# haosulab/ActiveZero

Measured on AMD Instinct MI355X. Metric: stereo pairs/sec (540x960, D=192) fwd+bwd, higher is better.
Workload: dtype f32; 1 GPU; configs[1]: PSMNet 540x960 (padded to 544 rows) D=192 fwd+bwd+Adam, supervised disparity loss, batch 4 per GPU; global_batch=4, height=540, width=960, maxdisp=192, parallelism=dp1

## Files before the change

activezero_amd/conv3d.py:

```python
import collections
import os

import torch

from . import _lib, overlap, packing, profiler
from .amax import AMAX_SLOTS, ZEROS, absmax, _get_amax, _set_amax, weight_amax
from .handover import slot_contribute, slot_leftover, slot_register, sum_parts
from .ops import _call, _chk, _p, _stream

CONV_S1, CONV_S2, DECONV_S2 = 0, 1, 2
FP32, BF16X6, F16X3 = 0, 1, 3
_PREC = {"fp32": FP32, "bf16x6": BF16X6, "f16x3": F16X3}
_BWD_F16 = os.environ.get("AZ_BWD_F16", "1") != "0"
PRESPLIT = os.environ.get("AZ_PRESPLIT", "1") != "0"
BF16X6_R16 = 2
_ROLL = os.environ.get("AZ_CONV_ROLL", "1") != "0"


_OFF32 = 0xffffff00


def _fits32(x, cin, cout):
    if isinstance(x, LazyCostVolume):
        return True
    _, d, h, w, _ = x.shape
    return d * h * w * max(cin, cout) * 4 < _OFF32


def _fits32_transposed(x, op_cin, op_cout):
    if not (op_cin == 64 and op_cout == 32):
        return True
    _, d, h, w, _ = x.shape
    return d * h * w * 64 * 4 < _OFF32 and 8 * d * h * w * 32 * 4 < _OFF32


def _layout(precision, mode, op_cout, fits32=True):
    if precision == BF16X6 and mode == CONV_S1 and op_cout == 32 and _ROLL and fits32:
        return BF16X6_R16
    return precision


def _fwd_launch(weight, mode):
    if mode == DECONV_S2:
        cin, cout = weight.shape[0], weight.shape[1]
        return cin, cout, 27, cout * 27
    cout, cin = weight.shape[0], weight.shape[1]
    return cin, cout, cin * 27, 27


def _dgrad_launch(mode, cin, cout):
    if mode == CONV_S1:
        return CONV_S1, cout, cin, 27, cin * 27, True
    if mode == CONV_S2:
        return DECONV_S2, cout, cin, 27, cin * 27, False
    return CONV_S2, cout, cin, cout * 27, 27, False


def _f16_fwd_ok(mode, cin, cout):
    return cin in (32, 64) and cout in (32, 64)


def _f16_dgrad_ok(mode, cin, cout):
    return _f16_fwd_ok(*_dgrad_launch(mode, cin, cout)[:3])


def _f16_wgrad_ok(mode, cin, cout):
    return cin in (32, 64) and cout in (32, 64)


def _f16_launch_ok(op_mode, ci, co, operand):
    if not _f16_fwd_ok(op_mode, ci, co):
        return False
    if op_mode == DECONV_S2:
        return _fits32_transposed(operand, ci, co)
    if _fits32(operand, ci, co):
        return True
    if op_mode == CONV_S1:
        return not (co == 32 or ci == co == 64)
    return not (ci == 32 and co == 64 and _lib.lib().az_option(b"AZ_CONV_S2ROLL") != 0)


class Arith(collections.namedtuple("Arith", "conv wgrad sink bwd16", defaults=(None, False))):
    __slots__ = ()

    @classmethod
    def of(cls, conv="bf16x6", wgrad=None, bwd16=None):
        w = wgrad if wgrad is not None else conv
        if bwd16 is None:
            bwd16 = _BWD_F16 or conv == "f16x3"
        return cls(_PREC[conv], BF16X6 if w == "f16x3" else _PREC[w], None, bool(bwd16) and conv != "fp32" and w != "fp32")

    @property
    def names(self):
        inv = {v: k for k, v in _PREC.items()}
        return inv[self.conv], ("f16x3" if self.bwd16 else inv[self.wgrad])


DEFAULT_ARITH = Arith.of(os.environ.get("AZ_CONV_PRECISION", "f16x3"), os.environ.get("AZ_WGRAD_PRECISION"))


def _arith(a):
    if a is None:
        return DEFAULT_ARITH
    if isinstance(a, str):
        return Arith.of(a)
    return a


def _dims(x):
    b, d, h, w, c = x.shape
    return b, d, h, w, c


def _out_dims(mode, d, h, w):
    if mode == CONV_S1:
        return d, h, w
    if mode == CONV_S2:
        return (d - 1) // 2 + 1, (h - 1) // 2 + 1, (w - 1) // 2 + 1
    return 2 * d, 2 * h, 2 * w


def _pack(weight, op_cin, op_cout, stride_out, stride_in, flip, precision, cache=False):
    w = _chk(weight.detach().contiguous(), "weight")

    def make():
        n = _lib.lib().az_conv3d_packed_floats(op_cin, op_cout, precision)
        packed = torch.empty(n, dtype=torch.float32, device=w.device)
        _call("az_conv3d_pack_weights", _p(packed), _p(w), op_cin, op_cout, stride_out, stride_in,
              int(flip), precision, _stream())
        packed.az_precision = precision
        return packed

    key = (packing.cache_key(weight), op_cin, op_cout, stride_out, stride_in, bool(flip), precision) if cache else None
    return packing.memo(packing.PACK_CACHE, key, make, (weight,), 256)


def eval_affine(bn, like, cache=False):
    c = bn.num_features
    src = (bn.weight, bn.bias, bn.running_mean, bn.running_var, bn.num_batches_tracked)

    def make():
        scale, shift = like.new_empty(c), like.new_empty(c)
        _call("az_bn3d_eval_affine", _p(scale), _p(shift), _p(bn.weight.detach()), _p(bn.bias.detach()),
              _p(bn.running_mean), _p(bn.running_var), float(bn.eps), c, _stream())
        return scale, shift

    return packing.memo(packing.AFFINE_CACHE, (packing.cache_key(*src), float(bn.eps)) if cache else None, make, src, 512)


def _pack_forward(weight, mode, precision, cache=False, lazy=False, fits32=True):
    cin, cout, s_out, s_in = _fwd_launch(weight, mode)
    if not lazy:
        precision = _layout(precision, mode, cout, fits32)
    return _pack(weight, cin, cout, s_out, s_in, False, precision, cache), cin, cout


def _peak(precision):
    if precision == F16X3:
        return _PEAK_F16
    return (157.3, "fp32 MFMA") if precision == FP32 else (2500.0 / 6.0, "bf16x6: bf16 MFMA peak / 6")


def _conv_flops(b, vox_out, cin, cout, mode):
    taps = 27.0 / 8.0 if mode == DECONV_S2 else 27.0
    return 2.0 * taps * cin * cout * b * vox_out


class LazyCostVolume:

    def __init__(self, feat_l_nhwc, feat_r_nhwc, ndisp):
        self.fl, self.fr, self.ndisp = _chk(feat_l_nhwc, "feat_l"), _chk(feat_r_nhwc, "feat_r"), int(ndisp)
        if self.fl.shape != self.fr.shape or self.fl.shape[-1] != 32:
            raise RuntimeError("fused cost volume expects two [B,h,w,32] feature maps")


def _run_gather(x, packed, mode, cin, cout, precision, scale=None, shift=None, residual=None, relu=False,
                stats=False, tag="conv3d"):
    if isinstance(x, LazyCostVolume):
        if stats or mode != CONV_S1 or cin != 64:
            raise RuntimeError("the fused cost-volume operand is only wired for the eval-mode dres0[0] conv")
        b, h, w, _ = x.fl.shape
        d = x.ndisp
        out = x.fl.new_empty(b, d, h, w, cout)
        with profiler.scope(f"{tag}_costvol_m0_{cin}_{cout}", flops=_conv_flops(b, d * h * w, cin, cout, mode),
                            peak=_peak(precision)):
            _call("az_conv3d_fwd", _p(out), _p(x.fl), _p(x.fr), _p(packed), _p(scale), _p(shift),
                  _p(residual), int(relu), mode, 1, getattr(packed, "az_precision", precision), b, cin, cout, d, h, w,
                  _stream())
        return out
    b, d, h, w, c = _dims(x)
    assert c == cin, (c, cin)
    precision = getattr(packed, "az_precision", precision)
    if mode == CONV_S2 and ((d % 2 and d != 1) or h % 2 or w % 2):
        raise RuntimeError("stride-2 layers need even D/H/W (as PSMNet's hourglass does; D = 1: a 2-D layer)")
    do, ho, wo = _out_dims(mode, d, h, w)
    out = x.new_empty(b, do, ho, wo, cout)
    flops = _conv_flops(b, do * ho * wo, cin, cout, mode)
    name = f"{tag}_m{mode}_{cin}_{cout}"
    if stats:
        ntiles = _lib.lib().az_conv3d_stats_tiles(mode, precision, b, cin, cout, d, h, w)
        if ntiles <= 0:
            raise RuntimeError(f"az_conv3d_stats_tiles: {ntiles}")
        part = x.new_empty(cout, ntiles, 2)
        cnt = x.new_empty(ntiles)
        with profiler.scope(name, flops=flops, peak=_peak(precision)):
            _call("az_conv3d_fwd_stats", _p(out), _p(part), _p(cnt), _p(x), None, _p(packed), mode, 0,
                  precision, b, cin, cout, d, h, w, _stream())
        return out, part, cnt, ntiles
    with profiler.scope(name, flops=flops, peak=_peak(precision)):
        _call("az_conv3d_fwd", _p(out), _p(x), None, _p(packed), _p(scale), _p(shift), _p(residual),
              int(relu), mode, 0, precision, b, cin, cout, d, h, w, _stream())
    return out


_PEAK_F16 = (2500.0 / 3.0, "f16x3: fp16 MFMA peak / 3")


def _pack_f16(weight, op_cin, op_cout, stride_out, stride_in, flip, mode, cache=False):
    w = _chk(weight.detach().contiguous(), "weight")

    def pack_now(packed, w_amax):
        _call("az_conv3d_pack_weights_f16", _p(packed), _p(w), _p(w_amax), op_cin, op_cout, stride_out, stride_in,
              int(flip), mode, _stream())

    def make():
        w_amax = weight_amax(weight, w)
        packed = torch.empty(_lib.lib().az_conv3d_packed_floats_f16(op_cin, op_cout), dtype=torch.float32, device=w.device)
        pack_now(packed, w_amax)
        return packed, w_amax

    if cache:
        key = (packing.cache_key(weight), op_cin, op_cout, stride_out, stride_in, bool(flip), F16X3, mode)
        return packing.memo(packing.PACK_CACHE, key, make, (weight,), 256)
    kind = _lib.lib().az_conv3d_f16_layout(mode, op_cin, op_cout)
    if kind < 0:
        raise RuntimeError(f"az_conv3d_f16_layout({mode}, {op_cin}, {op_cout}): {kind}")
    hit = packing.planned_pack(weight, w, kind, op_cin, op_cout, op_cin, op_cout, stride_out, stride_in, 27, flip, pack_now)
    return hit if hit is not None else make()


def _is_split(t):
    return getattr(t, "az_split", False)


def _run_f16(x, packed, w_amax, mode, cin, cout, scale=None, shift=None, residual=None, relu=False, stats=False,
             tag="conv3d"):
    b, d, h, w, c = _dims(x)
    assert c == cin, (c, cin)
    do, ho, wo = _out_dims(mode, d, h, w)
    out = x.new_empty(b, do, ho, wo, cout)
    name = f"{tag}_m{mode}_{cin}_{cout}"
    flops = _conv_flops(b, do * ho * wo, cin, cout, mode)
    split = _is_split(x)
    x_amax = _get_amax(x) if split else absmax(x)
    if split and (stats or x_amax is None):
        raise RuntimeError("a pre-split tensor reached a launch that cannot read it")
    if stats:
        ntiles = _lib.lib().az_conv3d_stats_tiles_f16(mode, b, cin, cout, d, h, w)
        if ntiles <= 0:
            raise RuntimeError(f"az_conv3d_stats_tiles_f16: {ntiles}")
        part, cnt = x.new_empty(cout, ntiles, 2), x.new_empty(ntiles)
        with profiler.scope(name, flops=flops, peak=_PEAK_F16):
            _call("az_conv3d_fwd_stats_f16", _p(out), _p(part), _p(cnt), _p(x), _p(packed), _p(x_amax), _p(w_amax),
                  mode, b, cin, cout, d, h, w, _stream())
        return out, part, cnt, ntiles
    with profiler.scope(name, flops=flops, peak=_PEAK_F16):
        _call("az_conv3d_fwd_f16", _p(out), _p(x), _p(packed), _p(x_amax), _p(w_amax), int(split), _p(scale), _p(shift),
              _p(residual), int(relu), mode, b, cin, cout, d, h, w, _stream())
    return out


def _conv(x, weight, mode, precision, scale=None, shift=None, residual=None, relu=False, stats=False, cache=False,
          tag="conv3d"):
    lazy = isinstance(x, LazyCostVolume)
    cin, cout, s_out, s_in = _fwd_launch(weight, mode)
    if precision == F16X3 and not lazy and _f16_launch_ok(mode, cin, cout, x):
        pk, w_amax = _pack_f16(weight, cin, cout, s_out, s_in, False, mode, cache)
        return _run_f16(x, pk, w_amax, mode, cin, cout, scale, shift, residual, relu, stats, tag)
    prec = BF16X6 if precision == F16X3 else precision
    packed, cin, cout = _pack_forward(weight, mode, prec, cache=cache, lazy=lazy, fits32=_fits32(x, cin, cout))
    return _run_gather(x, packed, mode, cin, cout, prec, scale, shift, residual, relu, stats, tag)


def _wgrad_f16(coarse, fine, stride, cm, cn, tag, sink=None, late_ok=True):
    b, dc, hc, wc, _ = _dims(coarse)
    _, df, hf, wf, _ = _dims(fine)
    gw = coarse.new_empty(cm, cn, 3, 3, 3)
    ws_bytes = _lib.lib().az_conv3d_wgrad_workspace(cm, cn)
    am_c, am_f = _get_amax(coarse), _get_amax(fine)
    mask = (1 if _is_split(coarse) else 0) | (2 if _is_split(fine) else 0)
    if (mask & 1 and am_c is None) or (mask & 2 and am_f is None):
        raise RuntimeError("a pre-split tensor without its producer's amax")
    with overlap.scope(sink, coarse, fine, gw, am_c, am_f):
        late = late_ok and sink is not None and sink.live and overlap.DEFER_UNPACK
        ws = sink.take_workspace(ws_bytes // 4) if late else coarse.new_empty(ws_bytes // 4)
        am_c = am_c if mask & 1 else absmax(coarse)
        am_f = am_f if mask & 2 else absmax(fine)
        with profiler.scope(f"{tag}_wgrad_s{stride}_{cm}_{cn}", flops=2.0 * 27 * cm * cn * b * dc * hc * wc,
                            peak=_PEAK_F16):
            _call("az_conv3d_wgrad_f16", None if late else _p(gw), _p(ws), ws_bytes, _p(coarse), _p(fine), _p(am_c), _p(am_f),
                  mask, stride, b, cm, cn, dc, hc, wc, df, hf, wf, _stream())
        if late:
            sink.defer_unpack(gw, ws, cm, cn, cm, cn, 27)
        if sink is not None and sink.live:
            sink.keep.extend((am_c, am_f))
    return gw


def _weight_grad_f16(x, dy, mode, cin, cout, sink=None, late_ok=True):
    if mode == DECONV_S2:
        return _wgrad_f16(x, dy, 2, cin, cout, "deconv", sink, late_ok)
    return _wgrad_f16(dy, x, 1 if mode == CONV_S1 else 2, cout, cin, "conv", sink, late_ok)


def _wgrad(coarse, fine, stride, cm, cn, tag, precision, sink=None):
    b, dc, hc, wc, _ = _dims(coarse)
    _, df, hf, wf, _ = _dims(fine)
    gw = coarse.new_empty(cm, cn, 3, 3, 3)
    ws_bytes = _lib.lib().az_conv3d_wgrad_workspace(cm, cn)
    with overlap.scope(sink, coarse, fine, gw):
        ws = coarse.new_empty(ws_bytes // 4)
        with profiler.scope(f"{tag}_wgrad_s{stride}_{cm}_{cn}", flops=2.0 * 27 * cm * cn * b * dc * hc * wc,
                            peak=_peak(precision)):
            _call("az_conv3d_wgrad", _p(gw), _p(ws), ws_bytes, _p(coarse), _p(fine), stride, precision,
                  b, cm, cn, dc, hc, wc, df, hf, wf, _stream())
    return gw


def _input_grad(dy, weight, mode, cin, cout, precision, residual=None):
    op, ci, co, s_out, s_in, flip = _dgrad_launch(mode, cin, cout)
    if precision == F16X3:
        if _f16_launch_ok(op, ci, co, dy):
            pk, w_amax = _pack_f16(weight, ci, co, s_out, s_in, flip, op)
            return _run_f16(dy, pk, w_amax, op, ci, co, residual=residual, tag="dgrad")
        precision = BF16X6
    pk = _pack(weight, ci, co, s_out, s_in, flip, _layout(precision, op, co, _fits32(dy, ci, co)))
    return _run_gather(dy, pk, op, ci, co, precision, residual=residual, tag="dgrad")


def _weight_grad(x, dy, mode, cin, cout, precision, sink=None, late_ok=True):
    if precision == F16X3:
        if _f16_wgrad_ok(mode, cin, cout):
            return _weight_grad_f16(x, dy, mode, cin, cout, sink, late_ok)
        precision = BF16X6
    if mode == DECONV_S2:
        return _wgrad(x, dy, 2, cin, cout, "deconv", precision, sink)
    return _wgrad(dy, x, 1 if mode == CONV_S1 else 2, cout, cin, "conv", precision, sink)


def _presplit_ok(x, raw, mode, cin, cout, need_gx, need_gw):
    lib = _lib.lib()
    b, d, h, w, _ = raw.shape
    if need_gx:
        op, ci, co = _dgrad_launch(mode, cin, cout)[:3]
        if not _f16_launch_ok(op, ci, co, raw) or lib.az_conv3d_fwd_f16_split_ok(op, b, ci, co, d, h, w) != 1:
            return False
    if need_gw:
        if not _f16_wgrad_ok(mode, cin, cout):
            return False
        _, dx_, hx, wx, _ = x.shape
        if mode == DECONV_S2:
            ok, bit = lib.az_conv3d_wgrad_f16_split_ok(2, b, cin, cout, dx_, hx, wx, d, h, w), 2
        else:
            ok, bit = lib.az_conv3d_wgrad_f16_split_ok(1 if mode == CONV_S1 else 2, b, cout, cin, d, h, w, dx_, hx, wx), 1
        if not ok & bit:
            return False
    return bool(need_gx or need_gw)


class _ConvBN(torch.autograd.Function):

    @staticmethod
    def forward(ctx, x, weight, gamma, beta, residual, bn, mode, relu, arith, defer=None, x_slot=None, res_slot=None):
        ctx.x_slot, ctx.res_slot = x_slot, res_slot
        x = _chk(x, "x")
        if residual is not None:
            residual = _chk(residual, "residual")
        training = bn.training or not bn.track_running_stats
        eps = float(bn.eps)
        cin, cout = _fwd_launch(weight, mode)[:2]
        with torch.cuda.device(x.device):
            if not training:
                scale, shift = eval_affine(bn, x)
                raw = _conv(x, weight, mode, arith.conv)
                y = torch.empty_like(raw)
                y_amax = ZEROS.take(raw)
                _call("az_bn3d_apply", _p(y), _p(raw), _p(scale), _p(shift), _p(residual), int(relu),
                      raw.numel() // cout, cout, _p(y_amax), _stream())
                _set_amax(y, y_amax)
                ctx.save_for_backward(x, weight, gamma, raw, y if relu else None, bn.running_mean.clone(),
                                      scale, None, None)
                ctx.cfg = (mode, relu, residual is not None, cin, cout, arith, False)
                return y
            raw, part, cnt, ntiles = _conv(x, weight, mode, arith.conv, stats=True)
            scale, shift = x.new_empty(cout), x.new_empty(cout)
            mean, invstd = x.new_empty(cout), x.new_empty(cout)
            track = bn.track_running_stats and bn.running_mean is not None
            momentum = 0.1 if bn.momentum is None else float(bn.momentum)
            nbt = bn.num_batches_tracked if (track and bn.num_batches_tracked is not None) else None
            scratch = x.new_empty(int(_lib.lib().az_bn3d_finalize_scratch(cout))) if ntiles >= 4096 else None
            _call("az_bn3d_finalize", _p(mean), _p(invstd), _p(scale), _p(shift),
                  _p(bn.running_mean) if track else None, _p(bn.running_var) if track else None,
                  _p(part), _p(cnt), _p(gamma.detach()), _p(beta.detach()), ntiles, cout, eps,
                  momentum, _p(nbt), _p(scratch), scratch.numel() if scratch is not None else 0, _stream())
            if nbt is not None:
                packing.touched(nbt, bn.running_mean, bn.running_var)
            nvox = raw.numel() // cout
            if defer is not None and relu and residual is None:
                defer.scale, defer.shift = scale, shift
                y = raw
            else:
                y = torch.empty_like(raw)
                y_amax = ZEROS.take(raw)
                with profiler.scope(f"bn3d_apply_{cout}", bytes=4.0 * raw.numel() * (3 if residual is not None else 2),
                                    bound="hbm"):
                    _call("az_bn3d_apply", _p(y), _p(raw), _p(scale), _p(shift), _p(residual), int(relu),
                          nvox, cout, _p(y_amax), _stream())
                _set_amax(y, y_amax)
        remask = relu and residual is None
        ctx.save_for_backward(x, weight, gamma, raw, y if (relu and not remask) else None, mean, invstd,
                              scale if remask else None, shift if remask else None)
        if arith.sink is not None and not arith.sink.owns(weight):
            arith = arith._replace(sink=None)
        ctx.cfg = (mode, relu, residual is not None, cin, cout, arith, True)
        ctx.x_amax = _get_amax(x)
        return y

    @staticmethod
    def backward(ctx, gy):
        x, weight, gamma, raw, y, mean, invstd, scale, shift = ctx.saved_tensors
        mode, relu, has_res, cin, cout, arith, training = ctx.cfg
        gy = _chk(gy.contiguous(), "grad_y")
        nvox = raw.numel() // cout
        with torch.cuda.device(gy.device):
            gy = slot_leftover(ctx, gy)
            if not training:
                s_, rm = invstd, mean
                dz = gy * (y > 0).to(gy.dtype) if relu else gy
                dbeta = dz.sum(dim=(0, 1, 2, 3))
                rinv = torch.where(gamma.detach() != 0, s_ / gamma.detach(), torch.zeros_like(s_))
                dgamma = (dz * (raw - rm)).sum(dim=(0, 1, 2, 3)) * rinv
                dx_raw = (dz * s_).contiguous()
                g_res = dz if has_res else None
            else:
                lib = _lib.lib()
                dx_raw = torch.empty_like(raw)
                dz = torch.empty_like(raw) if (has_res and relu) else None
                dgamma, dbeta = gy.new_empty(cout), gy.new_empty(cout)
                coef = gy.new_empty(cout, 3)
                ws_bytes = lib.az_bn3d_bwd_workspace(nvox, cout)
                ws = gy.new_empty(ws_bytes // 4)
                dx_amax = gy.new_empty(AMAX_SLOTS) if arith.bwd16 else None
                split = arith.bwd16 and PRESPLIT and _presplit_ok(x, raw, mode, cin, cout, ctx.needs_input_grad[0],
                                                                  ctx.needs_input_grad[1])
                with profiler.scope(f"bn3d_bwd_{cout}", bytes=4.0 * raw.numel() * (7 if (relu and y is not None) else 5), bound="hbm"):
                    _call("az_bn3d_bwd", _p(dx_raw), _p(dz), _p(dgamma), _p(dbeta), _p(coef), _p(ws), ws_bytes,
                          _p(gy), _p(y), _p(raw), _p(mean), _p(invstd), _p(gamma.detach()), _p(scale), _p(shift),
                          int(relu), nvox, cout, _p(dx_amax), int(split), _stream())
                if dx_amax is not None:
                    _set_amax(dx_raw, dx_amax)
                if split:
                    dx_raw.az_split = True
                g_res = (dz if relu else gy) if has_res else None
            gx = gw = None
            if has_res:
                g_res = slot_contribute(ctx.res_slot, plain=g_res)
            if ctx.needs_input_grad[0]:
                gx = slot_contribute(ctx.x_slot, make=lambda r: _input_grad(dx_raw, weight, mode, cin, cout,
                                                                             F16X3 if arith.bwd16 else arith.conv, r))
            if ctx.needs_input_grad[1]:
                if getattr(ctx, "x_amax", None) is not None and _get_amax(x) is None:
                    _set_amax(x, ctx.x_amax)
                gw = _weight_grad(x, dx_raw, mode, cin, cout, F16X3 if arith.bwd16 else arith.wgrad, arith.sink)
        return gx, gw, dgamma, dbeta, g_res, None, None, None, None, None, None, None


class DeferredAffine:

    def __init__(self):
        self.scale = self.shift = None

    @property
    def pending(self):
        return self.scale is not None


def conv_bn(x, conv, bn, mode, relu=False, residual=None, arith=None, defer=None):
    arith = _arith(arith)
    if isinstance(x, LazyCostVolume):
        if torch.is_grad_enabled() or bn.training:
            raise RuntimeError("LazyCostVolume is an inference-only operand")
        with torch.cuda.device(x.fl.device):
            scale, shift = eval_affine(bn, x.fl, cache=True)
            return _conv(x, conv.weight, mode, arith.conv, scale, shift, residual, relu, cache=True)
    training = bn.training or not bn.track_running_stats
    if not training and not torch.is_grad_enabled():
        x = _chk(x, "x")
        with torch.cuda.device(x.device):
            scale, shift = eval_affine(bn, x, cache=True)
            return _conv(x, conv.weight, mode, arith.conv, scale, shift,
                         _chk(residual, "residual") if residual is not None else None, relu, cache=True)
    w = arith.sink.weight(conv.weight) if arith.sink is not None else conv.weight
    x_slot = slot_register(x)
    res_slot = slot_register(residual) if residual is not None else None
    return _ConvBN.apply(x, w, bn.weight, bn.bias, residual, bn, mode, relu, arith, defer, x_slot, res_slot)


class _ConvLogits(torch.autograd.Function):

    @staticmethod
    def forward(ctx, x, weight, addend, sink, scale=None, shift=None):
        ctx.sink = sink if (sink is not None and sink.owns(weight)) else None
        x = _chk(x, "x")
        w = _chk(weight.detach().contiguous(), "weight")
        b, d, h, wd, c = _dims(x)
        if c != 32 or tuple(w.shape) != (1, 32, 3, 3, 3):
            raise RuntimeError("classifier conv expects 32 -> 1 channels, 3x3x3")
        if addend is not None:
            addend = _chk(addend.contiguous(), "addend")
        out = x.new_empty(b, d, h, wd)
        with torch.cuda.device(x.device):
            with profiler.scope("conv3d_c1_fwd", bytes=4.0 * (x.numel() + out.numel()), bound="hbm"):
                _call("az_conv3d_c1_fwd", _p(out), _p(x), _p(w), _p(addend), _p(scale), _p(shift), b, d, h, wd, _stream())
        ctx.save_for_backward(x, w, scale, shift)
        ctx.has_add = addend is not None
        return out

    @staticmethod
    def backward(ctx, g):
        x, w, scale, shift = ctx.saved_tensors
        g = _chk(g.contiguous(), "grad_logits")
        b, d, h, wd, _ = _dims(x)
        gx = gw = None
        with torch.cuda.device(g.device):
            if ctx.needs_input_grad[0]:
                gx = torch.empty_like(x)
                with profiler.scope("conv3d_c1_dgrad", bytes=4.0 * (x.numel() + g.numel()), bound="hbm"):
                    _call("az_conv3d_c1_dgrad", _p(gx), _p(g), _p(w), b, d, h, wd, _stream())
            if ctx.needs_input_grad[1]:
                gw = torch.empty_like(w)
                with overlap.scope(ctx.sink, x, g, gw, scale, shift), \
                        profiler.scope("conv3d_c1_wgrad", bytes=4.0 * (x.numel() + g.numel()), bound="hbm"):
                    _call("az_conv3d_c1_wgrad", _p(gw), _p(x), _p(g), _p(scale), _p(shift), b, d, h, wd, _stream())
        return gx, gw, (g if ctx.has_add else None), None, None, None


def conv_logits(x, conv, addend=None, sink=None, affine=None):
    sc, sh = (affine.scale, affine.shift) if (affine is not None and affine.pending) else (None, None)
    return _ConvLogits.apply(x, sink.weight(conv.weight) if sink is not None else conv.weight, addend, sink, sc, sh)


class _AddRelu(torch.autograd.Function):
    @staticmethod
    def forward(ctx, a, b):
        a, b = _chk(a, "a"), _chk(b, "b")
        y = torch.empty_like(a)
        y_amax = ZEROS.take(a)
        with torch.cuda.device(a.device):
            _call("az_add_relu", _p(y), _p(a), _p(b), 0, a.numel(), _p(y_amax), _stream())
        _set_amax(y, y_amax)
        return y

    @staticmethod
    def backward(ctx, g):
        return g, g


def add(a, b):
    return _AddRelu.apply(a, b)


class _FanOut(torch.autograd.Function):

    @staticmethod
    def forward(ctx, x, n):
        views = tuple(x.view_as(x) for _ in range(n))
        am = _get_amax(x)
        if am is not None:
            for v in views:
                _set_amax(v, am)
        return views

    @staticmethod
    def backward(ctx, *grads):
        gs = [_chk(g.contiguous(), "grad") for g in grads if g is not None]
        if not gs:
            return None, None
        with torch.cuda.device(gs[0].device):
            return sum_parts(gs), None


def fanout(x, n):
    if not (torch.is_grad_enabled() and x.requires_grad) or x.numel() % 4:
        return (x,) * n
    return _FanOut.apply(x, n)


def conv_plain(x, weight, mode, arith=None):
    arith = _arith(arith)
    return _conv(_chk(x, "x"), weight, mode, arith.conv)
```

activezero_amd/csrc/az_bn3d.hip:

```cpp
#include <stdlib.h>

#include "az_roll_common.h"

__device__ __forceinline__ double bn_wave_sum(double v) {
#pragma unroll
    for (int o = 32; o > 0; o >>= 1) v += __shfl_xor(v, o);
    return v;
}
template <int NT>
__device__ __forceinline__ double bn_block_sum(double v, double *slots ) {
    v = bn_wave_sum(v);
    __syncthreads();
    if ((threadIdx.x & 63) == 0) slots[threadIdx.x >> 6] = v;
    __syncthreads();
    double t = 0.0;
#pragma unroll
    for (int w = 0; w < NT / 64; ++w) t += slots[w];
    return t;
}

#define BN_PRE_SLICES 32
__global__ void __launch_bounds__(256)
bn_premerge_kernel(float *__restrict__ part_out, float *__restrict__ cnt_out, const float *__restrict__ part,
                   const float *__restrict__ cnt, long long ntiles) {
    const int c = blockIdx.x, sl = blockIdx.y;
    const long long per = (ntiles + BN_PRE_SLICES - 1) / BN_PRE_SLICES;
    const long long t0 = sl * per, t1 = t0 + per < ntiles ? t0 + per : ntiles;
    __shared__ double slots[256 / 64];
    const float2 *pc = reinterpret_cast<const float2 *>(part) + (long long)c * ntiles;
    double n = 0.0, sum = 0.0;
    for (long long t = t0 + threadIdx.x; t < t1; t += 256) {
        n += (double)cnt[t];
        sum += (double)pc[t].x;
    }
    const double N = bn_block_sum<256>(n, slots);
    const double S = bn_block_sum<256>(sum, slots);
    const double mean = N > 0.0 ? S / N : 0.0;
    double m2 = 0.0;
    for (long long t = t0 + threadIdx.x; t < t1; t += 256) {
        const float nt = cnt[t];
        if (nt <= 0.f) continue;
        const float2 pr = pc[t];
        const double dlt = (double)pr.x / (double)nt - mean;
        m2 += (double)pr.y + (double)nt * dlt * dlt;
    }
    const double M2 = bn_block_sum<256>(m2, slots);
    if (threadIdx.x == 0) {
        reinterpret_cast<float2 *>(part_out)[c * BN_PRE_SLICES + sl] = make_float2((float)S, (float)M2);
        if (c == 0) cnt_out[sl] = (float)N;
    }
}

#define BN_FIN_THREADS 1024
__global__ void __launch_bounds__(BN_FIN_THREADS)
bn_finalize_kernel(float *__restrict__ mean_out, float *__restrict__ invstd_out,
                   float *__restrict__ scale, float *__restrict__ shift,
                   float *__restrict__ running_mean, float *__restrict__ running_var,
                   const float *__restrict__ part, const float *__restrict__ cnt,
                   const float *__restrict__ gamma, const float *__restrict__ beta,
                   long long ntiles, int C, float eps, float momentum, int groups,
                   long long *__restrict__ num_batches_tracked) {
    const int c = blockIdx.x;
    if (num_batches_tracked != nullptr && c == 0 && threadIdx.x == 0) *num_batches_tracked += groups;
    for (int grp = 0; grp < groups; ++grp, part += (long long)C * ntiles * 2, cnt += ntiles,
             mean_out += C, invstd_out += C, scale += C, shift += C) {
    __shared__ double slots[BN_FIN_THREADS / 64];
    const float2 *pc = reinterpret_cast<const float2 *>(part) + (long long)c * ntiles;
    double n = 0.0, sum = 0.0;
    for (long long t = threadIdx.x; t < ntiles; t += BN_FIN_THREADS) {
        n += (double)cnt[t];
        sum += (double)pc[t].x;
    }
    const double Ntot = bn_block_sum<BN_FIN_THREADS>(n, slots);
    const double mean_all = bn_block_sum<BN_FIN_THREADS>(sum, slots) / Ntot;
    double m2 = 0.0;
    for (long long t = threadIdx.x; t < ntiles; t += BN_FIN_THREADS) {
        const float nt = cnt[t];
        if (nt <= 0.f) continue;
        const float2 pr = pc[t];
        const double dlt = (double)pr.x / (double)nt - mean_all;
        m2 += (double)pr.y + (double)nt * dlt * dlt;
    }
    const double M2 = bn_block_sum<BN_FIN_THREADS>(m2, slots);
    if (threadIdx.x == 0) {
        const double N = Ntot, mu = mean_all, var = M2 / N;
        const double istd = 1.0 / sqrt(var + (double)eps);
        mean_out[c] = (float)mu;
        invstd_out[c] = (float)istd;
        const float sc = gamma[c] * (float)istd;
        scale[c] = sc;
        shift[c] = beta[c] - (float)mu * sc;
        if (running_mean) {
            const double unbiased = N > 1.0 ? M2 / (N - 1.0) : var;
            running_mean[c] = (1.f - momentum) * running_mean[c] + momentum * (float)mu;
            running_var[c] = (1.f - momentum) * running_var[c] + momentum * (float)unbiased;
        }
    }
    }
}

__global__ void bn_eval_affine_kernel(float *scale, float *shift, const float *gamma,
                                      const float *beta, const float *rm, const float *rv,
                                      float eps, int C) {
    const int c = blockIdx.x * blockDim.x + threadIdx.x;
    if (c >= C) return;
    const float sc = gamma[c] / sqrtf(rv[c] + eps);
    scale[c] = sc;
    shift[c] = beta[c] - rm[c] * sc;
}

typedef float az_v4f __attribute__((ext_vector_type(4)));
template <bool NT>
__device__ __forceinline__ float4 bn_ld4(const float4 *p) {
    if (NT) {
        const az_v4f v = __builtin_nontemporal_load(reinterpret_cast<const az_v4f *>(p));
        return make_float4(v[0], v[1], v[2], v[3]);
    }
    return *p;
}
template <bool NT>
__device__ __forceinline__ void bn_st4(float4 *p, const float4 &o) {
    if (NT) {
        const az_v4f v = {o.x, o.y, o.z, o.w};
        __builtin_nontemporal_store(v, reinterpret_cast<az_v4f *>(p));
    } else {
        *p = o;
    }
}
#define BN_NT_BYTES (256LL << 20)

template <int C, bool NT>
__global__ void __launch_bounds__(256)
bn_apply_kernel(float4 *__restrict__ y, const float4 *__restrict__ x,
                const float *__restrict__ scale, const float *__restrict__ shift,
                const float4 *__restrict__ res, int relu, long long total4, unsigned *__restrict__ amax = nullptr) {
    constexpr int C4 = C / 4;
    unsigned am = 0;
    __shared__ float4 ssc[C4], ssh[C4];
    {
        const long long go = (long long)blockIdx.y * total4;
        y += go; x += go; if (res) res += go;
        scale += blockIdx.y * C; shift += blockIdx.y * C;
    }
    if (threadIdx.x < C4) {
        ssc[threadIdx.x] = reinterpret_cast<const float4 *>(scale)[threadIdx.x];
        ssh[threadIdx.x] = reinterpret_cast<const float4 *>(shift)[threadIdx.x];
    }
    __syncthreads();
    for (long long i = blockIdx.x * 256LL + threadIdx.x; i < total4; i += gridDim.x * 256LL) {
        const int c4 = (int)(i % C4);
        const float4 v = bn_ld4<NT>(&x[i]), sc = ssc[c4], sh = ssh[c4];
        float4 o = make_float4(fmaf(v.x, sc.x, sh.x), fmaf(v.y, sc.y, sh.y), fmaf(v.z, sc.z, sh.z),
                               fmaf(v.w, sc.w, sh.w));
        if (res) {
            const float4 r = bn_ld4<NT>(&res[i]);
            o.x += r.x; o.y += r.y; o.z += r.z; o.w += r.w;
        }
        if (relu) {
            o.x = fmaxf(o.x, 0.f); o.y = fmaxf(o.y, 0.f); o.z = fmaxf(o.z, 0.f); o.w = fmaxf(o.w, 0.f);
        }
        bn_st4<NT>(&y[i], o);
        az_amax_acc(am, o);
    }
    if (amax) az_amax_flush(amax, am);
}

__device__ __forceinline__ int c4_of(int tid, int C4) { return tid % C4; }

template <int C, bool NT>
__global__ void __launch_bounds__(256)
bn_bwd_reduce_kernel(float *__restrict__ partial, const float *__restrict__ dy,
                     const float *__restrict__ y, const float *__restrict__ x,
                     const float *__restrict__ mean, const float *__restrict__ invstd,
                     const float *__restrict__ scale, const float *__restrict__ shift, int relu,
                     long long nvox, unsigned *__restrict__ amax_zero = nullptr, unsigned *__restrict__ pmax = nullptr) {
    if (amax_zero && blockIdx.x == 0 && blockIdx.y == 0 && threadIdx.x < AZ_AMAX_SLOTS) amax_zero[threadIdx.x * AZ_AMAX_STRIDE] = 0u;
    constexpr int C4 = C / 4, VPB = 256 / C4;
    const bool remask = relu && scale != nullptr;
    {
        const long long go = (long long)blockIdx.y * nvox * C;
        dy += go; x += go; if (relu && !remask) y += go;
        mean += blockIdx.y * C; invstd += blockIdx.y * C;
        if (remask) { scale += blockIdx.y * C; shift += blockIdx.y * C; }
        partial += (size_t)blockIdx.y * gridDim.x * C * 2;
    }
    float4 sc = make_float4(0, 0, 0, 0), sh = sc;
    if (remask) { sc = reinterpret_cast<const float4 *>(scale)[c4_of(threadIdx.x, C4)]; sh = reinterpret_cast<const float4 *>(shift)[c4_of(threadIdx.x, C4)]; }
    const int c4 = threadIdx.x % C4, vl = threadIdx.x / C4;
    const float4 mu = reinterpret_cast<const float4 *>(mean)[c4];
    const float4 is = reinterpret_cast<const float4 *>(invstd)[c4];
    float4 s1 = make_float4(0, 0, 0, 0), s2 = make_float4(0, 0, 0, 0);
    uint4 mg = make_uint4(0, 0, 0, 0), mx = make_uint4(0, 0, 0, 0);
    auto body = [&](const float4 gin, const float4 xx, const float4 yin, float4 &t1, float4 &t2) {
        float4 g = gin;
        if (relu) {
            float4 yy = yin;
            if (remask) yy = make_float4(fmaf(xx.x, sc.x, sh.x), fmaf(xx.y, sc.y, sh.y), fmaf(xx.z, sc.z, sh.z), fmaf(xx.w, sc.w, sh.w));
            g.x = yy.x > 0.f ? g.x : 0.f; g.y = yy.y > 0.f ? g.y : 0.f;
            g.z = yy.z > 0.f ? g.z : 0.f; g.w = yy.w > 0.f ? g.w : 0.f;
        }
        const float4 xh = make_float4((xx.x - mu.x) * is.x, (xx.y - mu.y) * is.y, (xx.z - mu.z) * is.z, (xx.w - mu.w) * is.w);
        t1.x += g.x; t1.y += g.y; t1.z += g.z; t1.w += g.w;
        t2.x += g.x * xh.x; t2.y += g.y * xh.y; t2.z += g.z * xh.z; t2.w += g.w * xh.w;
        if (pmax) {
            mg.x = max(mg.x, az_finite_abs_bits(g.x)); mg.y = max(mg.y, az_finite_abs_bits(g.y));
            mg.z = max(mg.z, az_finite_abs_bits(g.z)); mg.w = max(mg.w, az_finite_abs_bits(g.w));
            mx.x = max(mx.x, az_finite_abs_bits(xh.x)); mx.y = max(mx.y, az_finite_abs_bits(xh.y));
            mx.z = max(mx.z, az_finite_abs_bits(xh.z)); mx.w = max(mx.w, az_finite_abs_bits(xh.w));
        }
    };
    const long long stride = (long long)gridDim.x * VPB;
    float4 u1 = make_float4(0, 0, 0, 0), u2 = make_float4(0, 0, 0, 0);
    const float4 zero4 = make_float4(0, 0, 0, 0);
    long long v = (long long)blockIdx.x * VPB + vl;
    for (; v + stride < nvox; v += 2 * stride) {
        const size_t i = (size_t)v * C4 + c4, i2 = (size_t)(v + stride) * C4 + c4;
        const float4 ga = bn_ld4<NT>(reinterpret_cast<const float4 *>(dy) + i), gb = bn_ld4<NT>(reinterpret_cast<const float4 *>(dy) + i2);
        const float4 xa = bn_ld4<NT>(reinterpret_cast<const float4 *>(x) + i), xb = bn_ld4<NT>(reinterpret_cast<const float4 *>(x) + i2);
        float4 ya = zero4, yb = zero4;
        if (relu && !remask) { ya = bn_ld4<NT>(reinterpret_cast<const float4 *>(y) + i); yb = bn_ld4<NT>(reinterpret_cast<const float4 *>(y) + i2); }
        body(ga, xa, ya, s1, s2);
        body(gb, xb, yb, u1, u2);
    }
    if (v < nvox) {
        const size_t i = (size_t)v * C4 + c4;
        const float4 ga = bn_ld4<NT>(reinterpret_cast<const float4 *>(dy) + i), xa = bn_ld4<NT>(reinterpret_cast<const float4 *>(x) + i);
        float4 ya = zero4;
        if (relu && !remask) ya = bn_ld4<NT>(reinterpret_cast<const float4 *>(y) + i);
        body(ga, xa, ya, s1, s2);
    }
    s1.x += u1.x; s1.y += u1.y; s1.z += u1.z; s1.w += u1.w;
    s2.x += u2.x; s2.y += u2.y; s2.z += u2.z; s2.w += u2.w;
    static_assert(C4 <= 64 && 64 % C4 == 0, "channel quads must tile a wave");
#pragma unroll
    for (int off = C4; off < 64; off <<= 1) {
        s1.x += __shfl_xor(s1.x, off); s1.y += __shfl_xor(s1.y, off); s1.z += __shfl_xor(s1.z, off); s1.w += __shfl_xor(s1.w, off);
        s2.x += __shfl_xor(s2.x, off); s2.y += __shfl_xor(s2.y, off); s2.z += __shfl_xor(s2.z, off); s2.w += __shfl_xor(s2.w, off);
    }
    __shared__ float4 r1[4][C4], r2[4][C4];
    const int wave = threadIdx.x >> 6, lane = threadIdx.x & 63;
    if (lane < C4) { r1[wave][lane] = s1; r2[wave][lane] = s2; }
    __syncthreads();
    if (threadIdx.x < C4) {
#pragma unroll
        for (int k = 1; k < 4; ++k) {
            const float4 a = r1[k][c4], b = r2[k][c4];
            s1.x += a.x; s1.y += a.y; s1.z += a.z; s1.w += a.w;
            s2.x += b.x; s2.y += b.y; s2.z += b.z; s2.w += b.w;
        }
        float *p = partial + ((size_t)blockIdx.x * C + c4 * 4) * 2;
        p[0] = s1.x; p[1] = s2.x; p[2] = s1.y; p[3] = s2.y;
        p[4] = s1.z; p[5] = s2.z; p[6] = s1.w; p[7] = s2.w;
    }
    if (pmax) {
#pragma unroll
        for (int off = C4; off < 64; off <<= 1) {
            mg.x = max(mg.x, (unsigned)__shfl_xor((int)mg.x, off)); mg.y = max(mg.y, (unsigned)__shfl_xor((int)mg.y, off));
            mg.z = max(mg.z, (unsigned)__shfl_xor((int)mg.z, off)); mg.w = max(mg.w, (unsigned)__shfl_xor((int)mg.w, off));
            mx.x = max(mx.x, (unsigned)__shfl_xor((int)mx.x, off)); mx.y = max(mx.y, (unsigned)__shfl_xor((int)mx.y, off));
            mx.z = max(mx.z, (unsigned)__shfl_xor((int)mx.z, off)); mx.w = max(mx.w, (unsigned)__shfl_xor((int)mx.w, off));
        }
        __shared__ uint4 q1[4][C4], q2[4][C4];
        if (lane < C4) { q1[wave][lane] = mg; q2[wave][lane] = mx; }
        __syncthreads();
        if (threadIdx.x < C4) {
#pragma unroll
            for (int k = 1; k < 4; ++k) {
                const uint4 a = q1[k][c4], b = q2[k][c4];
                mg.x = max(mg.x, a.x); mg.y = max(mg.y, a.y); mg.z = max(mg.z, a.z); mg.w = max(mg.w, a.w);
                mx.x = max(mx.x, b.x); mx.y = max(mx.y, b.y); mx.z = max(mx.z, b.z); mx.w = max(mx.w, b.w);
            }
            unsigned *p = pmax + ((size_t)blockIdx.y * gridDim.x * C + (size_t)blockIdx.x * C + c4 * 4) * 2;
            p[0] = mg.x; p[1] = mx.x; p[2] = mg.y; p[3] = mx.y;
            p[4] = mg.z; p[5] = mx.z; p[6] = mg.w; p[7] = mx.w;
        }
    }
}

#define BN_BWD_PARTIAL_FLOATS 32768
template <int C, bool NT>
__global__ void __launch_bounds__(256)
bn_bwd_apply_kernel(float4 *__restrict__ dx, float4 *__restrict__ dz_out,
                    const float4 *__restrict__ dy, const float4 *__restrict__ y,
                    const float4 *__restrict__ x, const float *__restrict__ mean,
                    const float *__restrict__ invstd, float *__restrict__ coef,
                    const float *__restrict__ scale, const float *__restrict__ shift, int relu,
                    long long total4, const float *__restrict__ partial, int nblocks, const float *__restrict__ gamma,
                    float *__restrict__ dgamma, float *__restrict__ dbeta, double nvox,
                    unsigned *__restrict__ amax = nullptr, const unsigned *__restrict__ pmax = nullptr) {
    constexpr int C4 = C / 4;
    unsigned am = 0;
    float split_scale = 1.f;
    __shared__ float smu[C], sis[C], k0[C], k1[C], k2[C], ssc[C], ssh[C];
    const bool remask = relu && scale != nullptr;
    const int grp = blockIdx.y;
    {
        const long long go = (long long)grp * total4;
        dx += go; dy += go; x += go; if (relu && !remask) y += go; if (dz_out) dz_out += go;
        mean += grp * C; invstd += grp * C; coef += grp * C * 3;
        if (remask) { scale += grp * C; shift += grp * C; }
    }
    if (remask && threadIdx.x < C) { ssc[threadIdx.x] = scale[threadIdx.x]; ssh[threadIdx.x] = shift[threadIdx.x]; }
    if (threadIdx.x < C) {
        smu[threadIdx.x] = mean[threadIdx.x];
        sis[threadIdx.x] = invstd[threadIdx.x];
    }
    constexpr int COLS = C / 2, ROWS = 256 / COLS;
    static_assert(COLS <= 64 && 64 % COLS == 0, "a partial row must tile a wave");
    __shared__ float wsum[4][2 * C];
    const int j = threadIdx.x % COLS, r = threadIdx.x / COLS, wave = threadIdx.x >> 6;
    const bool writer = blockIdx.x == 0;
    const int g_lo = (writer && grp == 0) ? 0 : grp, g_hi = (writer && grp == 0) ? (int)gridDim.y : grp + 1;
    double dg_tot = 0.0, db_tot = 0.0;
    for (int g = g_lo; g < g_hi; ++g) {
        const float4 *p4 = reinterpret_cast<const float4 *>(partial) + (size_t)g * nblocks * COLS;
        double a0 = 0.0, a1 = 0.0, a2 = 0.0, a3 = 0.0;
        for (int blk = r; blk < nblocks; blk += ROWS) {
            const float4 v = p4[(size_t)blk * COLS + j];
            a0 += v.x; a1 += v.y; a2 += v.z; a3 += v.w;
        }
#pragma unroll
        for (int off = COLS; off < 64; off <<= 1) {
            a0 += __shfl_xor(a0, off); a1 += __shfl_xor(a1, off); a2 += __shfl_xor(a2, off); a3 += __shfl_xor(a3, off);
        }
        __syncthreads();
        if ((threadIdx.x & 63) < COLS) {
            wsum[wave][4 * j + 0] = (float)a0; wsum[wave][4 * j + 1] = (float)a1;
            wsum[wave][4 * j + 2] = (float)a2; wsum[wave][4 * j + 3] = (float)a3;
        }
        __syncthreads();
        if (threadIdx.x < C) {
            const int c = threadIdx.x;
            const double sa = ((double)wsum[0][2 * c] + (double)wsum[1][2 * c]) + ((double)wsum[2][2 * c] + (double)wsum[3][2 * c]);
            const double sb = ((double)wsum[0][2 * c + 1] + (double)wsum[1][2 * c + 1]) + ((double)wsum[2][2 * c + 1] + (double)wsum[3][2 * c + 1]);
            db_tot += sa; dg_tot += sb;
            if (g == grp) {
                k0[c] = gamma[c] * sis[c];
                k1[c] = (float)(sa / nvox);
                k2[c] = (float)(sb / nvox);
                if (writer) { coef[c * 3 + 0] = k0[c]; coef[c * 3 + 1] = k1[c]; coef[c * 3 + 2] = k2[c]; }
            }
        }
    }
    if (writer && grp == 0 && threadIdx.x < C) { dbeta[threadIdx.x] = (float)db_tot; dgamma[threadIdx.x] = (float)dg_tot; }
    if (pmax) {
        const uint4 *m4 = reinterpret_cast<const uint4 *>(pmax);
        uint4 m = make_uint4(0, 0, 0, 0);
        for (int blk = r; blk < nblocks; blk += ROWS) {
            const uint4 v = m4[(size_t)blk * COLS + j];
            m.x = max(m.x, v.x); m.y = max(m.y, v.y); m.z = max(m.z, v.z); m.w = max(m.w, v.w);
        }
#pragma unroll
        for (int off = COLS; off < 64; off <<= 1) {
            m.x = max(m.x, (unsigned)__shfl_xor((int)m.x, off)); m.y = max(m.y, (unsigned)__shfl_xor((int)m.y, off));
            m.z = max(m.z, (unsigned)__shfl_xor((int)m.z, off)); m.w = max(m.w, (unsigned)__shfl_xor((int)m.w, off));
        }
        __syncthreads();
        if ((threadIdx.x & 63) < COLS) {
            wsum[wave][4 * j + 0] = __uint_as_float(m.x); wsum[wave][4 * j + 1] = __uint_as_float(m.y);
            wsum[wave][4 * j + 2] = __uint_as_float(m.z); wsum[wave][4 * j + 3] = __uint_as_float(m.w);
        }
        __syncthreads();
        float bnd = 0.f;
        if (threadIdx.x < C) {
            const int c = threadIdx.x;
            const float gm = fmaxf(fmaxf(wsum[0][2 * c], wsum[1][2 * c]), fmaxf(wsum[2][2 * c], wsum[3][2 * c]));
            const float xm = fmaxf(fmaxf(wsum[0][2 * c + 1], wsum[1][2 * c + 1]), fmaxf(wsum[2][2 * c + 1], wsum[3][2 * c + 1]));
            bnd = fabsf(k0[c]) * (gm + fabsf(k1[c]) + xm * fabsf(k2[c])) * 1.000001f;
            bnd = bnd < __builtin_inff() ? bnd : 0.f;
        }
#pragma unroll
        for (int off = 32; off > 0; off >>= 1) bnd = fmaxf(bnd, __shfl_xor(bnd, off));
        __shared__ float bwave[4];
        if ((threadIdx.x & 63) == 0) bwave[wave] = bnd;
        __syncthreads();
        bnd = fmaxf(fmaxf(bwave[0], bwave[1]), fmaxf(bwave[2], bwave[3]));
        split_scale = az_pow2(az_f16_scale_exp(bnd));
        if (writer && grp == 0 && threadIdx.x == 0 && amax) amax[0] = __float_as_uint(bnd);
    }
    __syncthreads();
    for (long long i = blockIdx.x * 256LL + threadIdx.x; i < total4; i += gridDim.x * 256LL) {
        const int c = (int)(i % C4) * 4;
        float4 g = bn_ld4<NT>(&dy[i]);
        const float4 xx = bn_ld4<NT>(&x[i]);
        if (relu) {
            float4 yy;
            if (remask) yy = make_float4(fmaf(xx.x, ssc[c + 0], ssh[c + 0]), fmaf(xx.y, ssc[c + 1], ssh[c + 1]),
                                         fmaf(xx.z, ssc[c + 2], ssh[c + 2]), fmaf(xx.w, ssc[c + 3], ssh[c + 3]));
            else yy = bn_ld4<NT>(&y[i]);
            g.x = yy.x > 0.f ? g.x : 0.f; g.y = yy.y > 0.f ? g.y : 0.f;
            g.z = yy.z > 0.f ? g.z : 0.f; g.w = yy.w > 0.f ? g.w : 0.f;
        }
        if (dz_out) bn_st4<NT>(&dz_out[i], g);
        float4 o;
        o.x = k0[c + 0] * (g.x - k1[c + 0] - (xx.x - smu[c + 0]) * sis[c + 0] * k2[c + 0]);
        o.y = k0[c + 1] * (g.y - k1[c + 1] - (xx.y - smu[c + 1]) * sis[c + 1] * k2[c + 1]);
        o.z = k0[c + 2] * (g.z - k1[c + 2] - (xx.z - smu[c + 2]) * sis[c + 2] * k2[c + 2]);
        o.w = k0[c + 3] * (g.w - k1[c + 3] - (xx.w - smu[c + 3]) * sis[c + 3] * k2[c + 3]);
        if (pmax) {
            bn_st4<NT>(&dx[i], az_presplit_f16x4(make_float4(o.x * split_scale, o.y * split_scale, o.z * split_scale, o.w * split_scale)));
        } else {
            bn_st4<NT>(&dx[i], o);
            az_amax_acc(am, o);
        }
    }
    if (amax && !pmax) az_amax_flush(amax, am);
}

__global__ void __launch_bounds__(256)
add_relu_kernel(float4 *__restrict__ y, const float4 *__restrict__ a,
                const float4 *__restrict__ b, int relu, long long total4, unsigned *__restrict__ amax) {
    unsigned am = 0;
    for (long long i = blockIdx.x * 256LL + threadIdx.x; i < total4; i += gridDim.x * 256LL) {
        const float4 p = a[i], q = b[i];
        float4 o = make_float4(p.x + q.x, p.y + q.y, p.z + q.z, p.w + q.w);
        if (relu) {
            o.x = fmaxf(o.x, 0.f); o.y = fmaxf(o.y, 0.f); o.z = fmaxf(o.z, 0.f); o.w = fmaxf(o.w, 0.f);
        }
        y[i] = o;
        az_amax_acc(am, o);
    }
    if (amax) az_amax_flush(amax, am);
}


template <int C>
__global__ void __launch_bounds__(256)
bn_stats_kernel(float *__restrict__ part, float *__restrict__ cnt, const float *__restrict__ x,
                long long nvox, long long ntiles) {
    constexpr int C4 = C / 4, VPB = 256 / C4;
    const int c4 = threadIdx.x % C4, vl = threadIdx.x / C4;
    x += (size_t)blockIdx.y * nvox * C;
    part += (size_t)blockIdx.y * C * ntiles * 2;
    cnt += (size_t)blockIdx.y * ntiles;
    const long long v0 = (long long)blockIdx.x * VPB;
    const float4 K = reinterpret_cast<const float4 *>(x)[(size_t)v0 * C4 + c4];
    float4 s1 = make_float4(0, 0, 0, 0), s2 = make_float4(0, 0, 0, 0);
    int n = 0;
    for (long long v = v0 + vl; v < nvox; v += (long long)gridDim.x * VPB) {
        const float4 a = reinterpret_cast<const float4 *>(x)[(size_t)v * C4 + c4];
        const float dx = a.x - K.x, dy = a.y - K.y, dz = a.z - K.z, dw = a.w - K.w;
        s1.x += dx; s1.y += dy; s1.z += dz; s1.w += dw;
        s2.x += dx * dx; s2.y += dy * dy; s2.z += dz * dz; s2.w += dw * dw;
        ++n;
    }
    __shared__ float4 r1[256], r2[256];
    __shared__ int rn[256];
    r1[threadIdx.x] = s1; r2[threadIdx.x] = s2; rn[threadIdx.x] = n;
    __syncthreads();
    if (vl == 0) {
        for (int k = 1; k < VPB; ++k) {
            const float4 a = r1[k * C4 + c4], b = r2[k * C4 + c4];
            s1.x += a.x; s1.y += a.y; s1.z += a.z; s1.w += a.w;
            s2.x += b.x; s2.y += b.y; s2.z += b.z; s2.w += b.w;
            n += rn[k * C4 + c4];
        }
        const float fn = (float)n;
        const float s[4] = {s1.x, s1.y, s1.z, s1.w}, q[4] = {s2.x, s2.y, s2.z, s2.w};
        const float k4[4] = {K.x, K.y, K.z, K.w};
#pragma unroll
        for (int e = 0; e < 4; ++e) {
            float2 o;
            o.x = s[e] + fn * k4[e];
            o.y = fmaxf(q[e] - s[e] * s[e] / fn, 0.f);
            reinterpret_cast<float2 *>(part)[(size_t)(c4 * 4 + e) * ntiles + blockIdx.x] = o;
        }
        if (c4 == 0) cnt[blockIdx.x] = fn;
    }
}

__global__ void __launch_bounds__(256)
sum4_kernel(float4 *__restrict__ y, const float4 *__restrict__ a, const float4 *__restrict__ b,
            const float4 *__restrict__ c, const float4 *__restrict__ d, long long total4) {
    for (long long i = blockIdx.x * 256LL + threadIdx.x; i < total4; i += gridDim.x * 256LL) {
        const float4 p = a[i], q = b[i];
        float4 o = make_float4(p.x + q.x, p.y + q.y, p.z + q.z, p.w + q.w);
        if (c) { const float4 r = c[i]; o.x += r.x; o.y += r.y; o.z += r.z; o.w += r.w; }
        if (d) { const float4 r = d[i]; o.x += r.x; o.y += r.y; o.z += r.z; o.w += r.w; }
        y[i] = o;
    }
}

#define BN_GRID(total) az_grid_for((total), 256)
static int bn_bwd_fused_blocks(int blocks, int C) {
    const int cap = BN_BWD_PARTIAL_FLOATS / (2 * C);
    return blocks < cap ? blocks : cap;
}
static unsigned bn_bwd_apply_grid(long long total4) {
    const unsigned g = az_grid_for(total4, 256);
    return g < 1024u ? g : 1024u;
}
#define BN_LAUNCH(KERNEL, C, NT, GRID, STREAM, ...)                                                             \
    do {                                                                                                        \
        if (NT) {                                                                                               \
            if ((C) == 32) hipLaunchKernelGGL((KERNEL<32, true>), GRID, dim3(256), 0, STREAM, __VA_ARGS__);     \
            else if ((C) == 64) hipLaunchKernelGGL((KERNEL<64, true>), GRID, dim3(256), 0, STREAM, __VA_ARGS__); \
            else hipLaunchKernelGGL((KERNEL<128, true>), GRID, dim3(256), 0, STREAM, __VA_ARGS__);              \
        } else {                                                                                                \
            if ((C) == 32) hipLaunchKernelGGL((KERNEL<32, false>), GRID, dim3(256), 0, STREAM, __VA_ARGS__);    \
            else if ((C) == 64) hipLaunchKernelGGL((KERNEL<64, false>), GRID, dim3(256), 0, STREAM, __VA_ARGS__); \
            else hipLaunchKernelGGL((KERNEL<128, false>), GRID, dim3(256), 0, STREAM, __VA_ARGS__);             \
        }                                                                                                       \
    } while (0)

extern "C" long long az_bn3d_finalize_scratch(int C) { return (long long)C * BN_PRE_SLICES * 2 + BN_PRE_SLICES; }

extern "C" int az_bn3d_finalize(float *mean, float *invstd, float *scale, float *shift,
                                float *running_mean, float *running_var, const float *partials,
                                const float *counts, const float *gamma, const float *beta,
                                long long ntiles, int C, float eps, float momentum,
                                long long *num_batches_tracked, float *scratch,
                                long long scratch_floats, void *stream) {
    AZ_REQUIRE_PTR(mean); AZ_REQUIRE_PTR(invstd); AZ_REQUIRE_PTR(scale); AZ_REQUIRE_PTR(shift);
    AZ_REQUIRE_PTR(partials); AZ_REQUIRE_PTR(counts); AZ_REQUIRE_PTR(gamma); AZ_REQUIRE_PTR(beta);
    AZ_REQUIRE(ntiles > 0 && C > 0);
    if ((running_mean == nullptr) != (running_var == nullptr)) return AZ_EINVAL;
    if (scratch != nullptr && ntiles >= 4096) {
        if (scratch_floats < az_bn3d_finalize_scratch(C)) return AZ_EWORKSPACE;
        float *p2 = scratch, *c2 = scratch + (size_t)C * BN_PRE_SLICES * 2;
        hipLaunchKernelGGL(bn_premerge_kernel, dim3(C, BN_PRE_SLICES), dim3(256), 0, az_stream(stream), p2, c2, partials,
                           counts, ntiles);
        partials = p2; counts = c2; ntiles = BN_PRE_SLICES;
    }
    hipLaunchKernelGGL(bn_finalize_kernel, dim3(C), dim3(BN_FIN_THREADS), 0, az_stream(stream), mean, invstd,
                       scale, shift, running_mean, running_var, partials, counts, gamma, beta,
                       ntiles, C, eps, momentum, 1, num_batches_tracked);
    return az_launch_status();
}

extern "C" int az_bn3d_eval_affine(float *scale, float *shift, const float *gamma,
                                   const float *beta, const float *running_mean,
                                   const float *running_var, float eps, int C, void *stream) {
    AZ_REQUIRE_PTR(scale); AZ_REQUIRE_PTR(shift); AZ_REQUIRE_PTR(gamma); AZ_REQUIRE_PTR(beta);
    AZ_REQUIRE_PTR(running_mean); AZ_REQUIRE_PTR(running_var);
    AZ_REQUIRE(C > 0);
    hipLaunchKernelGGL(bn_eval_affine_kernel, dim3((C + 63) / 64), dim3(64), 0, az_stream(stream),
                       scale, shift, gamma, beta, running_mean, running_var, eps, C);
    return az_launch_status();
}

extern "C" int az_bn3d_apply(float *y, const float *x, const float *scale, const float *shift,
                             const float *residual, int relu, long long nvox, int C, float *y_amax,
                             void *stream) {
    AZ_REQUIRE_PTR(y); AZ_REQUIRE_PTR(x); AZ_REQUIRE_PTR(scale); AZ_REQUIRE_PTR(shift);
    AZ_REQUIRE(nvox > 0);
    const long long total4 = nvox * C / 4;
    const float4 *r4 = reinterpret_cast<const float4 *>(residual);
    if (C != 32 && C != 64 && C != 128) return AZ_EUNSUPPORTED;
    const bool nt = total4 * 16 >= BN_NT_BYTES;
    BN_LAUNCH(bn_apply_kernel, C, nt, dim3(BN_GRID(total4)), az_stream(stream), (float4 *)y, (const float4 *)x, scale,
              shift, r4, relu, total4, reinterpret_cast<unsigned *>(y_amax));
    return az_launch_status();
}

static long long bn3d_bwd_blocks(long long nvox, int C) {
    const int vpb = 256 / (C / 4);
    return az_grid_for((nvox + vpb - 1) / vpb * 256, 256);
}
extern "C" long long az_bn3d_bwd_workspace(long long nvox, int C) {
    if (nvox <= 0 || (C != 32 && C != 64 && C != 128)) return AZ_EINVAL;
    return 2 * bn3d_bwd_blocks(nvox, C) * C * 2 * (long long)sizeof(float);
}

extern "C" int az_bn3d_bwd(float *dx, float *dz_out, float *dgamma, float *dbeta, float *coef,
                           float *workspace, long long workspace_bytes, const float *dy,
                           const float *y, const float *x, const float *mean,
                           const float *invstd, const float *gamma, const float *scale,
                           const float *shift, int relu, long long nvox, int C, float *dx_amax, int split_out,
                           void *stream) {
    unsigned *const am = reinterpret_cast<unsigned *>(dx_amax);
    AZ_REQUIRE_PTR(dx); AZ_REQUIRE_PTR(dgamma); AZ_REQUIRE_PTR(dbeta); AZ_REQUIRE_PTR(coef);
    AZ_REQUIRE_PTR(workspace); AZ_REQUIRE_PTR(dy); AZ_REQUIRE_PTR(x); AZ_REQUIRE_PTR(mean);
    AZ_REQUIRE_PTR(invstd); AZ_REQUIRE_PTR(gamma);
    if ((scale == nullptr) != (shift == nullptr)) return AZ_EINVAL;
    if (relu && !scale) AZ_REQUIRE_PTR(y);
    const long long need = az_bn3d_bwd_workspace(nvox, C);
    if (need < 0) return (int)need;
    if (workspace_bytes < need) return AZ_EWORKSPACE;
    int blocks = (int)bn3d_bwd_blocks(nvox, C);
    const long long total4 = nvox * C / 4;
    hipStream_t s = az_stream(stream);
    const bool nt = total4 * 16 >= BN_NT_BYTES;
    if (split_out && !am) return AZ_ENULL;
    blocks = bn_bwd_fused_blocks(blocks, C);
    unsigned *const pmax = split_out ? reinterpret_cast<unsigned *>(workspace) + (size_t)blocks * C * 2 : nullptr;
    BN_LAUNCH(bn_bwd_reduce_kernel, C, nt, dim3(blocks), s, workspace, dy, y, x, mean, invstd, scale, shift, relu, nvox, am, pmax);
    BN_LAUNCH(bn_bwd_apply_kernel, C, nt, dim3(bn_bwd_apply_grid(total4)), s, (float4 *)dx, (float4 *)dz_out, (const float4 *)dy,
              (const float4 *)y, (const float4 *)x, mean, invstd, coef, scale, shift, relu, total4,
              (const float *)workspace, blocks, gamma, dgamma, dbeta, (double)nvox, am, (const unsigned *)pmax);
    return az_launch_status();
}

extern "C" int az_add_relu(float *y, const float *a, const float *b, int relu, long long n, float *y_amax,
                           void *stream) {
    AZ_REQUIRE_PTR(y); AZ_REQUIRE_PTR(a); AZ_REQUIRE_PTR(b);
    AZ_REQUIRE(n > 0 && n % 4 == 0);
    hipLaunchKernelGGL(add_relu_kernel, dim3(BN_GRID(n / 4)), dim3(256), 0, az_stream(stream),
                       (float4 *)y, (const float4 *)a, (const float4 *)b, relu, n / 4, reinterpret_cast<unsigned *>(y_amax));
    return az_launch_status();
}

extern "C" int az_sum4(float *y, const float *a, const float *b, const float *c, const float *d, long long n,
                       void *stream) {
    AZ_REQUIRE_PTR(y); AZ_REQUIRE_PTR(a); AZ_REQUIRE_PTR(b);
    if (d && !c) return AZ_EINVAL;
    AZ_REQUIRE(n > 0 && n % 4 == 0);
    hipLaunchKernelGGL(sum4_kernel, dim3(BN_GRID(n / 4)), dim3(256), 0, az_stream(stream), (float4 *)y,
                       (const float4 *)a, (const float4 *)b, (const float4 *)c, (const float4 *)d, n / 4);
    return az_launch_status();
}

extern "C" long long az_bn3d_stats_tiles(long long nvox, int C) {
    if (nvox <= 0 || (C != 32 && C != 64 && C != 128)) return AZ_EINVAL;
    const int vpb = 256 / (C / 4);
    long long t = (nvox + (long long)vpb * 16 - 1) / ((long long)vpb * 16);
    if (t > 2048) t = 2048;
    if (t < 1) t = 1;
    return t;
}

extern "C" int az_bn3d_stats(float *partials, float *counts, const float *x, long long nvox, int C,
                             void *stream) {
    AZ_REQUIRE_PTR(partials); AZ_REQUIRE_PTR(counts); AZ_REQUIRE_PTR(x);
    const long long tiles = az_bn3d_stats_tiles(nvox, C);
    if (tiles < 0) return (int)tiles;
    hipStream_t s = az_stream(stream);
    if (C == 32)
        hipLaunchKernelGGL(bn_stats_kernel<32>, dim3((unsigned)tiles), dim3(256), 0, s, partials, counts, x, nvox, tiles);
    else if (C == 64)
        hipLaunchKernelGGL(bn_stats_kernel<64>, dim3((unsigned)tiles), dim3(256), 0, s, partials, counts, x, nvox, tiles);
    else
        hipLaunchKernelGGL(bn_stats_kernel<128>, dim3((unsigned)tiles), dim3(256), 0, s, partials, counts, x, nvox, tiles);
    return az_launch_status();
}

static int bn2d_blocks(long long nvox, int C) {
    const int vpb = 256 / (C / 4);
    return (int)az_grid_for((nvox + vpb - 1) / vpb * 256, 256);
}

extern "C" long long az_bn2d_workspace(int groups, long long nvox, int C) {
    const long long tiles = az_bn3d_stats_tiles(nvox, C);
    if (tiles < 0 || groups <= 0) return AZ_EINVAL;
    const long long fwd = (long long)groups * (C * tiles * 2 + tiles);
    const long long bwd = (long long)groups * ((long long)bn2d_blocks(nvox, C) * C * 2 + C * 3);
    return (fwd > bwd ? fwd : bwd) * (long long)sizeof(float);
}

template <int C>
static void bn2d_fwd_launch(float *y, float *mean, float *invstd, float *scale, float *shift, float *rm,
                            float *rv, const float *x, const float *res, const float *gamma,
                            const float *beta, float *ws, int relu, int groups, long long nvox, float eps,
                            float momentum, long long *nbt, const float *pre_part, const float *pre_cnt,
                            long long pre_tiles, hipStream_t s, unsigned *amax) {
    long long tiles = az_bn3d_stats_tiles(nvox, C);
    const float *part = ws, *cnt = ws + (size_t)groups * C * tiles * 2;
    if (pre_part != nullptr) {
        part = pre_part; cnt = pre_cnt; tiles = pre_tiles;
    } else {
        hipLaunchKernelGGL(bn_stats_kernel<C>, dim3((unsigned)tiles, groups), dim3(256), 0, s, ws,
                           ws + (size_t)groups * C * tiles * 2, x, nvox, tiles);
    }
    hipLaunchKernelGGL(bn_finalize_kernel, dim3(C), dim3(BN_FIN_THREADS), 0, s, mean, invstd, scale, shift, rm, rv,
                       part, cnt, gamma, beta, tiles, C, eps, momentum, groups, nbt);
    const long long total4 = nvox * C / 4;
    hipLaunchKernelGGL((bn_apply_kernel<C, false>), dim3(BN_GRID(total4), groups), dim3(256), 0, s, (float4 *)y,
                       (const float4 *)x, scale, shift, (const float4 *)res, relu, total4, amax);
}

extern "C" int az_bn2d_fwd(float *y, float *mean, float *invstd, float *scale, float *shift,
                           float *running_mean, float *running_var, const float *x, const float *residual,
                           const float *gamma, const float *beta, float *workspace, long long workspace_bytes,
                           int relu, int groups, long long nvox, int C, float eps, float momentum,
                           long long *num_batches_tracked, const float *partials,
                           const float *counts, long long partial_tiles, float *y_amax, void *stream) {
    unsigned *const am = reinterpret_cast<unsigned *>(y_amax);
    AZ_REQUIRE_PTR(y); AZ_REQUIRE_PTR(mean); AZ_REQUIRE_PTR(invstd); AZ_REQUIRE_PTR(scale); AZ_REQUIRE_PTR(shift);
    AZ_REQUIRE_PTR(x); AZ_REQUIRE_PTR(gamma); AZ_REQUIRE_PTR(beta); AZ_REQUIRE_PTR(workspace);
    if ((running_mean == nullptr) != (running_var == nullptr)) return AZ_EINVAL;
    if ((partials == nullptr) != (counts == nullptr) || (partials != nullptr && partial_tiles <= 0)) return AZ_EINVAL;
    const long long need = az_bn2d_workspace(groups, nvox, C);
    if (need < 0) return (int)need;
    if (workspace_bytes < need) return AZ_EWORKSPACE;
    if (groups > 65535) return AZ_EUNSUPPORTED;
    hipStream_t s = az_stream(stream);
    if (C == 32) bn2d_fwd_launch<32>(y, mean, invstd, scale, shift, running_mean, running_var, x, residual, gamma, beta, workspace, relu, groups, nvox, eps, momentum, num_batches_tracked, partials, counts, partial_tiles, s, am);
    else if (C == 64) bn2d_fwd_launch<64>(y, mean, invstd, scale, shift, running_mean, running_var, x, residual, gamma, beta, workspace, relu, groups, nvox, eps, momentum, num_batches_tracked, partials, counts, partial_tiles, s, am);
    else bn2d_fwd_launch<128>(y, mean, invstd, scale, shift, running_mean, running_var, x, residual, gamma, beta, workspace, relu, groups, nvox, eps, momentum, num_batches_tracked, partials, counts, partial_tiles, s, am);
    return az_launch_status();
}

template <int C>
static void bn2d_bwd_launch(float *dx, float *dz, float *dgamma, float *dbeta, float *ws, const float *dy,
                            const float *y, const float *x, const float *mean, const float *invstd,
                            const float *gamma, const float *scale, const float *shift, int relu, int groups,
                            long long nvox, hipStream_t s, unsigned *amax) {
    int blocks = bn2d_blocks(nvox, C);
    float *partial = ws, *coef = ws + (size_t)groups * blocks * C * 2;
    const long long total4 = nvox * C / 4;
    blocks = bn_bwd_fused_blocks(blocks, C);
    hipLaunchKernelGGL((bn_bwd_reduce_kernel<C, false>), dim3(blocks, groups), dim3(256), 0, s, partial, dy, y, x, mean,
                       invstd, scale, shift, relu, nvox);
    hipLaunchKernelGGL((bn_bwd_apply_kernel<C, false>), dim3(bn_bwd_apply_grid(total4), groups), dim3(256), 0, s, (float4 *)dx,
                       (float4 *)dz, (const float4 *)dy, (const float4 *)y, (const float4 *)x, mean, invstd,
                       coef, scale, shift, relu, total4, (const float *)partial, blocks, gamma, dgamma, dbeta, (double)nvox, amax);
}

extern "C" int az_bn2d_bwd(float *dx, float *dz_out, float *dgamma, float *dbeta, float *workspace,
                           long long workspace_bytes, const float *dy, const float *y, const float *x,
                           const float *mean, const float *invstd, const float *gamma, const float *scale,
                           const float *shift, int relu, int groups, long long nvox, int C, float *dx_amax,
                           void *stream) {
    AZ_REQUIRE_PTR(dx); AZ_REQUIRE_PTR(dgamma); AZ_REQUIRE_PTR(dbeta); AZ_REQUIRE_PTR(workspace);
    AZ_REQUIRE_PTR(dy); AZ_REQUIRE_PTR(x); AZ_REQUIRE_PTR(mean); AZ_REQUIRE_PTR(invstd); AZ_REQUIRE_PTR(gamma);
    if ((scale == nullptr) != (shift == nullptr)) return AZ_EINVAL;
    if (relu && !scale) AZ_REQUIRE_PTR(y);
    unsigned *const am = reinterpret_cast<unsigned *>(dx_amax);
    const long long need = az_bn2d_workspace(groups, nvox, C);
    if (need < 0) return (int)need;
    if (workspace_bytes < need) return AZ_EWORKSPACE;
    if (groups > 65535) return AZ_EUNSUPPORTED;
    hipStream_t s = az_stream(stream);
    if (C == 32) bn2d_bwd_launch<32>(dx, dz_out, dgamma, dbeta, workspace, dy, y, x, mean, invstd, gamma, scale, shift, relu, groups, nvox, s, am);
    else if (C == 64) bn2d_bwd_launch<64>(dx, dz_out, dgamma, dbeta, workspace, dy, y, x, mean, invstd, gamma, scale, shift, relu, groups, nvox, s, am);
    else bn2d_bwd_launch<128>(dx, dz_out, dgamma, dbeta, workspace, dy, y, x, mean, invstd, gamma, scale, shift, relu, groups, nvox, s, am);
    return az_launch_status();
}
```

activezero_amd/csrc/az_conv3d_c1.hip:

```cpp
#include "az_common.h"
#include "az_launch_math.h"

#define C1_TH 8
#define C1_TW 32
#define C1_VS 36
#define C1_GP 36
typedef float c1_f2 __attribute__((ext_vector_type(2)));
#define C1_FMA2(a, b, c) __builtin_elementwise_fma(a, b, c)


#define C1F_TH 8
#define C1F_TW 16
template <int CTRL>
__device__ __forceinline__ float c1_dpp_add(float v) {
    return v + __builtin_bit_cast(float, __builtin_amdgcn_update_dpp(0, __builtin_bit_cast(int, v), CTRL, 0xf, 0xf, true));
}
__global__ void __launch_bounds__(256)
c1_fwd_kernel(float *__restrict__ out, const float *__restrict__ in, const float *__restrict__ w,
              const float *__restrict__ addend, const float *__restrict__ in_scale,
              const float *__restrict__ in_shift, int D, int H, int W, int tiles_x, int dseg) {
    constexpr int SX = C1F_TW + 2, SY = C1F_TH + 2;
    __shared__ __attribute__((aligned(16))) float slab[SY * SX * C1_VS];
    const int tx0 = (blockIdx.x % tiles_x) * C1F_TW, ty0 = (blockIdx.x / tiles_x) * C1F_TH;
    const int d0 = blockIdx.y * dseg, d1 = min(d0 + dseg, D), b = blockIdx.z;
    const int cp = threadIdx.x & 15, grp = threadIdx.x >> 4;
    const int ly = grp >> 1, lx0 = (grp & 1) * 8;
    const int oh = ty0 + ly;
    c1_f2 wp[27];
#pragma unroll
    for (int t = 0; t < 27; ++t) wp[t] = c1_f2{w[(cp * 2 + 0) * 27 + t], w[(cp * 2 + 1) * 27 + t]};
    c1_f2 a_prev[8], a_cur[8], a_next[8];
#pragma unroll
    for (int j = 0; j < 8; ++j) { a_prev[j] = c1_f2{0.f, 0.f}; a_cur[j] = c1_f2{0.f, 0.f}; a_next[j] = c1_f2{0.f, 0.f}; }
    constexpr int NQ = SY * SX * 8, NLD = (NQ + 255) / 256;
    float4 pre[NLD];
    const bool affine = in_scale != nullptr;
    float4 isc = make_float4(1.f, 1.f, 1.f, 1.f), ish = make_float4(0.f, 0.f, 0.f, 0.f);
    if (affine) {
        isc = reinterpret_cast<const float4 *>(in_scale)[threadIdx.x & 7];
        ish = reinterpret_cast<const float4 *>(in_shift)[threadIdx.x & 7];
    }
    unsigned okbits = 0;
    auto issue = [&](int id) {
        okbits = 0;
#pragma unroll
        for (int it = 0; it < NLD; ++it) {
            const int q = threadIdx.x + 256 * it, v = q >> 3, part = q & 7;
            const int sy = v / SX, sx = v - sy * SX;
            const int ih = ty0 - 1 + sy, iw = tx0 - 1 + sx;
            pre[it] = make_float4(0.f, 0.f, 0.f, 0.f);
            if (q < NQ && id >= 0 && id < D && ih >= 0 && ih < H && iw >= 0 && iw < W) {
                pre[it] = *reinterpret_cast<const float4 *>(
                    in + ((((size_t)b * D + id) * H + ih) * W + iw) * 32 + part * 4);
                okbits |= 1u << it;
            }
        }
    };
    issue(d0 - 1);
    for (int id = d0 - 1; id <= d1; ++id) {
        if (id >= 0 && id < D) {
            __syncthreads();
#pragma unroll
            for (int it = 0; it < NLD; ++it) {
                const int q = threadIdx.x + 256 * it;
                float4 v = pre[it];
                if (affine && ((okbits >> it) & 1u)) {
                    v.x = fmaxf(fmaf(v.x, isc.x, ish.x), 0.f); v.y = fmaxf(fmaf(v.y, isc.y, ish.y), 0.f);
                    v.z = fmaxf(fmaf(v.z, isc.z, ish.z), 0.f); v.w = fmaxf(fmaf(v.w, isc.w, ish.w), 0.f);
                }
                if (q < NQ) *reinterpret_cast<float4 *>(&slab[(q >> 3) * C1_VS + (q & 7) * 4]) = v;
            }
            __syncthreads();
        }
        if (id < d1) issue(id + 1);
        if (id >= 0 && id < D) {
#pragma unroll
            for (int kh = 0; kh < 3; ++kh) {
                c1_f2 r[10];
                const float *row = &slab[((ly + kh) * SX + lx0) * C1_VS + cp * 2];
#pragma unroll
                for (int i = 0; i < 10; ++i) {
                    const float2 x = *reinterpret_cast<const float2 *>(row + i * C1_VS);
                    r[i] = c1_f2{x.x, x.y};
                }
#pragma unroll
                for (int kw = 0; kw < 3; ++kw)
#pragma unroll
                    for (int j = 0; j < 8; ++j) {
                        a_next[j] = C1_FMA2(r[j + kw], wp[kh * 3 + kw], a_next[j]);
                        a_cur[j] = C1_FMA2(r[j + kw], wp[9 + kh * 3 + kw], a_cur[j]);
                        a_prev[j] = C1_FMA2(r[j + kw], wp[18 + kh * 3 + kw], a_prev[j]);
                    }
            }
        }
        const int od = id - 1;
        if (od >= d0 && od < d1) {
            float mine = 0.f;
#pragma unroll
            for (int j = 0; j < 8; ++j) {
                float v = a_prev[j][0] + a_prev[j][1];
                v = c1_dpp_add<0xB1>(v);
                v = c1_dpp_add<0x4E>(v);
                v = c1_dpp_add<0x141>(v);
                v = c1_dpp_add<0x140>(v);
                mine = (cp == j) ? v : mine;
            }
            const int ow = tx0 + lx0 + cp;
            if (cp < 8 && oh < H && ow < W) {
                const size_t o = (((size_t)b * D + od) * H + oh) * W + ow;
                out[o] = addend ? mine + addend[o] : mine;
            }
        }
#pragma unroll
        for (int j = 0; j < 8; ++j) { a_prev[j] = a_cur[j]; a_cur[j] = a_next[j]; a_next[j] = c1_f2{0.f, 0.f}; }
    }
}

__device__ __forceinline__ void c1_load_gtile(float *gt, const float *__restrict__ gout, int b,
                                              int od, int ty0, int tx0, int D, int H, int W) {
    constexpr int SX = C1_TW + 2, SY = C1_TH + 2;
    for (int q = threadIdx.x; q < 3 * SY * SX; q += 256) {
        const int sx = q % SX;
        const int r = q / SX;
        const int sy = r % SY, sd = r / SY;
        const int gd = od - 1 + sd, gh = ty0 - 1 + sy, gw = tx0 - 1 + sx;
        gt[r * C1_GP + sx] = (gd >= 0 && gd < D && gh >= 0 && gh < H && gw >= 0 && gw < W)
                                 ? gout[(((size_t)b * D + gd) * H + gh) * W + gw] : 0.f;
    }
}
__device__ __forceinline__ void c1_row6(float (&r)[6], const float *gt, int pd, int sy, int lx0) {
    const float *row = static_cast<const float *>(__builtin_assume_aligned(gt + (pd * (C1_TH + 2) + sy) * C1_GP + lx0, 16));
    const float4 a = *reinterpret_cast<const float4 *>(row);
    const float2 c = *reinterpret_cast<const float2 *>(row + 4);
    r[0] = a.x; r[1] = a.y; r[2] = a.z; r[3] = a.w; r[4] = c.x; r[5] = c.y;
}

__global__ void __launch_bounds__(256)
c1_dgrad_kernel(float *__restrict__ gin, const float *__restrict__ gout,
                const float *__restrict__ w, int D, int H, int W, int tiles_x) {
    constexpr int SY = C1_TH + 2;
    __shared__ __attribute__((aligned(16))) float gt[3 * SY * C1_GP];
    const int tx0 = (blockIdx.x % tiles_x) * C1_TW, ty0 = (blockIdx.x / tiles_x) * C1_TH;
    const int od = blockIdx.y, b = blockIdx.z;
    c1_load_gtile(gt, gout, b, od, ty0, tx0, D, H, W);
    const int cp = threadIdx.x & 15, grp = threadIdx.x >> 4;
    c1_f2 wp[27];
#pragma unroll
    for (int t = 0; t < 27; ++t) wp[t] = c1_f2{w[(cp * 2 + 0) * 27 + t], w[(cp * 2 + 1) * 27 + t]};
    __syncthreads();
#pragma unroll 1
    for (int p = 0; p < C1_TH * C1_TW / 128; ++p) {
        const int gi = p * 16 + grp, ly = gi >> 2, lx0 = (gi & 3) * 8;
        const int oh = ty0 + ly;
        c1_f2 acc[8];
#pragma unroll
        for (int j = 0; j < 8; ++j) acc[j] = c1_f2{0.f, 0.f};
#pragma unroll
        for (int kd = 0; kd < 3; ++kd)
#pragma unroll
            for (int kh = 0; kh < 3; ++kh) {
                float r[12];
                {
                    const float *row = static_cast<const float *>(__builtin_assume_aligned(
                        gt + ((2 - kd) * SY + ly + 2 - kh) * C1_GP + lx0, 16));
                    const float4 a = *reinterpret_cast<const float4 *>(row);
                    const float4 c = *reinterpret_cast<const float4 *>(row + 4);
                    const float2 e = *reinterpret_cast<const float2 *>(row + 8);
                    r[0] = a.x; r[1] = a.y; r[2] = a.z; r[3] = a.w; r[4] = c.x; r[5] = c.y; r[6] = c.z; r[7] = c.w;
                    r[8] = e.x; r[9] = e.y;
                }
#pragma unroll
                for (int kw = 0; kw < 3; ++kw) {
                    const int t = (kd * 3 + kh) * 3 + kw;
#pragma unroll
                    for (int j = 0; j < 8; ++j) {
                        const c1_f2 g2 = {r[j + 2 - kw], r[j + 2 - kw]};
                        acc[j] = C1_FMA2(g2, wp[t], acc[j]);
                    }
                }
            }
#pragma unroll
        for (int j = 0; j < 8; ++j) asm volatile("" : "+v"(acc[j]));
        if (oh < H) {
            float *dst = gin + ((((size_t)b * D + od) * H + oh) * W + tx0 + lx0) * 32 + cp * 2;
#pragma unroll
            for (int j = 0; j < 8; ++j)
                if (tx0 + lx0 + j < W) *reinterpret_cast<float2 *>(dst + j * 32) = make_float2(acc[j][0], acc[j][1]);
        }
    }
}

__global__ void __launch_bounds__(256)
c1_wgrad_kernel(float *__restrict__ gw, const float *__restrict__ in,
                const float *__restrict__ gout, const float *__restrict__ in_scale,
                const float *__restrict__ in_shift, int D, int H, int W, int tiles_x, int tiles_y,
                long long ntiles) {
    constexpr int SY = C1_TH + 2;
    __shared__ __attribute__((aligned(16))) float gt[3 * SY * C1_GP];
    __shared__ float red[864];
    for (int q = threadIdx.x; q < 864; q += 256) red[q] = 0.f;
    const int quad = threadIdx.x & 7, grp = threadIdx.x >> 3;
    const bool affine = in_scale != nullptr;
    float4 isc = make_float4(1.f, 1.f, 1.f, 1.f), ish = make_float4(0.f, 0.f, 0.f, 0.f);
    if (affine) {
        isc = reinterpret_cast<const float4 *>(in_scale)[quad];
        ish = reinterpret_cast<const float4 *>(in_shift)[quad];
    }
    c1_f2 a01[27], a23[27];
#pragma unroll
    for (int t = 0; t < 27; ++t) { a01[t] = c1_f2{0.f, 0.f}; a23[t] = c1_f2{0.f, 0.f}; }
    for (long long item = blockIdx.x; item < ntiles; item += gridDim.x) {
        long long r = item;
        const int tx0 = (int)(r % tiles_x) * C1_TW; r /= tiles_x;
        const int ty0 = (int)(r % tiles_y) * C1_TH; r /= tiles_y;
        const int od = (int)(r % D);
        const int b = (int)(r / D);
        __syncthreads();
        c1_load_gtile(gt, gout, b, od, ty0, tx0, D, H, W);
        __syncthreads();
#pragma unroll 1
        for (int p = 0; p < C1_TH * C1_TW / 128; ++p) {
            const int gi = p * 32 + grp, ly = gi >> 3, lx0 = (gi & 7) * 4;
            const int ih = ty0 + ly;
            c1_f2 x01[4], x23[4];
            const float *src = in + ((((size_t)b * D + od) * H + ih) * W + tx0 + lx0) * 32 + quad * 4;
#pragma unroll
            for (int j = 0; j < 4; ++j) {
                float4 x = make_float4(0.f, 0.f, 0.f, 0.f);
                if (ih < H && tx0 + lx0 + j < W) {
                    x = *reinterpret_cast<const float4 *>(src + j * 32);
                    if (affine) {
                        x.x = fmaxf(fmaf(x.x, isc.x, ish.x), 0.f); x.y = fmaxf(fmaf(x.y, isc.y, ish.y), 0.f);
                        x.z = fmaxf(fmaf(x.z, isc.z, ish.z), 0.f); x.w = fmaxf(fmaf(x.w, isc.w, ish.w), 0.f);
                    }
                }
                x01[j] = c1_f2{x.x, x.y}; x23[j] = c1_f2{x.z, x.w};
            }
#pragma unroll
            for (int kd = 0; kd < 3; ++kd)
#pragma unroll
                for (int kh = 0; kh < 3; ++kh) {
                    float r[6];
                    c1_row6(r, gt, 2 - kd, ly + 2 - kh, lx0);
#pragma unroll
                    for (int kw = 0; kw < 3; ++kw) {
                        const int t = (kd * 3 + kh) * 3 + kw;
#pragma unroll
                        for (int j = 0; j < 4; ++j) {
                            const c1_f2 g2 = {r[j + 2 - kw], r[j + 2 - kw]};
                            a01[t] = C1_FMA2(g2, x01[j], a01[t]);
                            a23[t] = C1_FMA2(g2, x23[j], a23[t]);
                        }
                    }
                }
        }
    }
#pragma unroll
    for (int c = 0; c < 4; ++c)
#pragma unroll
        for (int t = 0; t < 27; ++t) {
            float v = (c < 2 ? a01[t] : a23[t])[c & 1];
            v += __shfl_xor(v, 8); v += __shfl_xor(v, 16); v += __shfl_xor(v, 32);
            if ((threadIdx.x & 63) < 8) atomicAdd(&red[(quad * 4 + c) * 27 + t], v);
        }
    __syncthreads();
    for (int q = threadIdx.x; q < 864; q += 256) atomicAdd(&gw[q], red[q]);
}

static int c1_check(int B, int D, int H, int W) {
    if (!(B > 0 && D > 0 && H > 0 && W > 0)) return AZ_EINVAL;
    if (B > 65535 || D > 65535) return AZ_EUNSUPPORTED;
    return AZ_OK;
}

extern "C" int az_conv3d_c1_fwd(float *logits, const float *in, const float *w,
                                const float *addend, const float *in_scale, const float *in_shift, int B, int D,
                                int H, int W, void *stream) {
    AZ_REQUIRE_PTR(logits); AZ_REQUIRE_PTR(in); AZ_REQUIRE_PTR(w);
    if ((in_scale == nullptr) != (in_shift == nullptr)) return AZ_EINVAL;
    if (int e = c1_check(B, D, H, W)) return e;
    const int tiles_x = (W + C1F_TW - 1) / C1F_TW, tiles_y = (H + C1F_TH - 1) / C1F_TH;
    const int best = az_c1_fwd_dseg((long long)tiles_x * tiles_y * B, D);
    hipLaunchKernelGGL(c1_fwd_kernel, dim3(tiles_x * tiles_y, (D + best - 1) / best, B), dim3(256), 0,
                       az_stream(stream), logits, in, w, addend, in_scale, in_shift, D, H, W, tiles_x, best);
    return az_launch_status();
}

extern "C" int az_conv3d_c1_dgrad(float *grad_in, const float *grad_logits, const float *w,
                                  int B, int D, int H, int W, void *stream) {
    AZ_REQUIRE_PTR(grad_in); AZ_REQUIRE_PTR(grad_logits); AZ_REQUIRE_PTR(w);
    if (int e = c1_check(B, D, H, W)) return e;
    const int tiles_x = (W + C1_TW - 1) / C1_TW, tiles_y = (H + C1_TH - 1) / C1_TH;
    hipLaunchKernelGGL(c1_dgrad_kernel, dim3(tiles_x * tiles_y, D, B), dim3(256), 0,
                       az_stream(stream), grad_in, grad_logits, w, D, H, W, tiles_x);
    return az_launch_status();
}

extern "C" int az_conv3d_c1_wgrad(float *grad_w, const float *in, const float *grad_logits,
                                  const float *in_scale, const float *in_shift, int B, int D, int H, int W,
                                  void *stream) {
    AZ_REQUIRE_PTR(grad_w); AZ_REQUIRE_PTR(in); AZ_REQUIRE_PTR(grad_logits);
    if ((in_scale == nullptr) != (in_shift == nullptr)) return AZ_EINVAL;
    if (int e = c1_check(B, D, H, W)) return e;
    if (hipMemsetAsync(grad_w, 0, 864 * sizeof(float), az_stream(stream)) != hipSuccess)
        return AZ_ELAUNCH;
    const int tiles_x = (W + C1_TW - 1) / C1_TW, tiles_y = (H + C1_TH - 1) / C1_TH;
    const long long ntiles = az_c1_wgrad_tiles(B, D, H, W);
    const unsigned grid = (unsigned)az_c1_wgrad_grid(ntiles);
    hipLaunchKernelGGL(c1_wgrad_kernel, dim3(grid), dim3(256), 0, az_stream(stream), grad_w, in,
                       grad_logits, in_scale, in_shift, D, H, W, tiles_x, tiles_y, ntiles);
    return az_launch_status();
}

extern "C" int az_conv3d_c1_plan(long long *plan, int B, int D, int H, int W) {
    AZ_REQUIRE_PTR(plan);
    if (int e = c1_check(B, D, H, W)) return e;
    const long long patches = (long long)((W + C1F_TW - 1) / C1F_TW) * ((H + C1F_TH - 1) / C1F_TH) * B;
    const int dseg = az_c1_fwd_dseg(patches, D);
    const long long ntiles = az_c1_wgrad_tiles(B, D, H, W);
    plan[0] = dseg;
    plan[1] = patches * ((D + dseg - 1) / dseg);
    plan[2] = ntiles;
    plan[3] = az_c1_wgrad_grid(ntiles);
    return AZ_OK;
}
```

include/azhip.h:

```cpp
#ifndef AZHIP_H
#define AZHIP_H

#include <stddef.h>
#include <stdint.h>

#ifdef __cplusplus
extern "C" {
#endif

#define AZ_OK 0
#define AZ_EINVAL (-1)
#define AZ_ENULL (-2)
#define AZ_ELAUNCH (-3)
#define AZ_EUNSUPPORTED (-4)
#define AZ_EWORKSPACE (-5)

const char *az_strerror(int code);
#define AZ_ABI_VERSION 6
int az_abi_version(void);
int az_option(const char *name);
int az_hbm_copy_probe(float *dst, const float *src, long long n, void *stream);

int az_warp_scatter(float *dst, const float *src, const int32_t *disp, int N, int C, int H,
                    int W, int sign, void *stream);

int az_cost_volume_fwd(float *cost, const float *feat_l, const float *feat_r, int B, int C,
                       int d, int h, int w, void *stream);
int az_cost_volume_bwd(float *grad_l, float *grad_r, const float *grad_cost, int B, int C,
                       int d, int h, int w, void *stream);
int az_cost_volume_fwd_ndhwc(float *cost, const float *feat_l, const float *feat_r, int B,
                             int C, int d, int h, int w, void *stream);
int az_cost_volume_bwd_ndhwc(float *grad_l, float *grad_r, const float *grad_cost, int B,
                             int C, int d, int h, int w, void *stream);

int az_softargmin_fwd(float *disp_out, float *stats_out, const float *logits, int B, int d, int h,
                      int w, void *stream);
int az_softargmin_bwd(float *grad_logits, const float *grad_disp, const float *logits,
                      const float *stats, const float *disp_fwd, int B, int d, int h, int w,
                      void *stream);

int az_warp_gather_fwd(float *out, const float *img, const float *disp, int B, int C, int H,
                       int W, void *stream);
int az_warp_gather_bwd(float *grad_disp, float *grad_img, const float *grad_out,
                       const float *img, const float *disp, int B, int C, int H, int W,
                       void *stream);

int az_patch_reproj_fwd(double *acc, const float *L, const float *R, const float *disp,
                        const uint8_t *mask, int B, int C, int H, int W, int ps, float sign,
                        void *stream);
int az_patch_reproj_bwd(float *grad_disp, const float *grad_loss, const double *acc,
                        const float *L, const float *R, const float *disp, const uint8_t *mask,
                        int B, int C, int H, int W, int ps, float sign, void *stream);
int az_patch_reproj_vis(float *vis, const float *R, const float *disp, int B, int C, int H,
                        int W, int ps, float sign, void *stream);

int az_lcn(float *normed, float *stdv, const float *img, int B, int H, int W, int ksize,
           float eps, long long img_batch_stride, void *stream);


long long az_conv3d_packed_floats(int cin, int cout, int precision);
int az_conv3d_pack_weights(float *packed, const float *w, int cin, int cout,
                           long long stride_out, long long stride_in, int flip, int precision,
                           void *stream);
long long az_conv3d_num_tiles(int mode, int B, int Di, int Hi, int Wi);
long long az_conv3d_stats_tiles(int mode, int precision, int B, int cin, int cout, int Di, int Hi, int Wi);
int az_conv3d_fwd(float *out, const float *in, const float *in2, const float *packed_w,
                  const float *scale, const float *shift, const float *residual, int relu,
                  int mode, int src, int precision, int B, int cin, int cout, int Di, int Hi,
                  int Wi, void *stream);
int az_conv3d_fwd_stats(float *out, float *partials, float *counts, const float *in,
                        const float *in2, const float *packed_w, int mode, int src,
                        int precision, int B, int cin, int cout, int Di, int Hi, int Wi,
                        void *stream);
long long az_conv3d_wgrad_workspace(int cm, int cn);
int az_conv3d_wgrad(float *grad_w, float *workspace, long long workspace_bytes,
                    const float *coarse, const float *fine, int stride, int precision, int B,
                    int cm, int cn, int Dc, int Hc, int Wc, int Df, int Hf, int Wf, void *stream);

#define AZ_AMAX_SLOTS 16
#define AZ_AMAX_STRIDE 64
#define AZ_AMAX_FLOATS (AZ_AMAX_SLOTS * AZ_AMAX_STRIDE)
int az_absmax(float *amax, const float *x, long long n, void *stream);
#define AZ_PACK_2D_SAME 0
#define AZ_PACK_2D_ROLL 1
#define AZ_PACK_3D_GATHER 2
#define AZ_PACK_3D_ROLL 3
#define AZ_PACK_3D_ROLL2 4
typedef struct AzPackDesc {
    void *dst;
    const float *src;
    const float *amax;
    long long s_co, s_ci;
    int kind, cin, cout, ci_real, co_real, taps, flip, pad_;
} AzPackDesc;
int az_pack_f16_multi(const AzPackDesc *descs, const int *block_desc, const int *first_block, int nd, int nblocks,
                      void *stream);
typedef struct AzUnpackDesc {
    float *dst;
    const float *ws;
    int cm, cn, cm_real, cn_real, taps, pad_;
} AzUnpackDesc;
int az_wgrad_unpack_multi(const AzUnpackDesc *descs, const int *block_desc, const int *first_block, int nd, int nblocks,
                          void *stream);
long long az_conv3d_packed_floats_f16(int cin, int cout);
int az_conv3d_pack_weights_f16(float *packed, const float *w, const float *w_amax, int cin, int cout,
                               long long stride_out, long long stride_in, int flip, int mode, void *stream);
int az_conv3d_f16_layout(int mode, int cin, int cout);
int az_conv3d_fwd_f16_split_ok(int mode, int B, int cin, int cout, int Di, int Hi, int Wi);
int az_conv3d_wgrad_f16_split_ok(int stride, int B, int cm, int cn, int Dc, int Hc, int Wc, int Df, int Hf, int Wf);
int az_conv3d_fwd_f16(float *out, const float *in, const float *packed_w, const float *in_amax,
                      const float *w_amax, int in_split, const float *scale, const float *shift, const float *residual,
                      int relu, int mode, int B, int cin, int cout, int Di, int Hi, int Wi, void *stream);
long long az_conv3d_stats_tiles_f16(int mode, int B, int cin, int cout, int Di, int Hi, int Wi);
int az_conv3d_fwd_stats_f16(float *out, float *partials, float *counts, const float *in, const float *packed_w,
                            const float *in_amax, const float *w_amax, int mode, int B, int cin, int cout,
                            int Di, int Hi, int Wi, void *stream);
int az_conv3d_wgrad_f16(float *grad_w, float *workspace, long long workspace_bytes, const float *coarse,
                        const float *fine, const float *coarse_amax, const float *fine_amax, int split_mask, int stride,
                        int B, int cm, int cn, int Dc, int Hc, int Wc, int Df, int Hf, int Wf, void *stream);

int az_conv2d_pack_weights_f16(float *packed, const float *w, const float *w_amax, int cin, int cout,
                               int ci_real, int co_real, long long stride_out, long long stride_in, int kh,
                               int kw, int flip, void *stream);
int az_conv2d_fwd_f16(float *out, const float *in, const float *packed_w, const float *in_amax,
                      const float *w_amax, const float *scale, const float *shift, const float *residual,
                      int relu, int B, int H, int W, int cin, int cout, int in_cstride, int out_cstride,
                      int res_cstride, int kh, int kw, int dilation, void *stream);
int az_conv2d_fwd_stats_f16(float *out, float *partials, float *counts, const float *in, const float *packed_w,
                            const float *in_amax, const float *w_amax, int groups, int B, int H, int W,
                            int cin, int cout, int in_cstride, int out_cstride, int kh, int kw, int dilation,
                            void *stream);
int az_conv2d_pack_weights_bf16_flipped(float *packed, const float *w, int cin, int cout, long long stride_out,
                                        long long stride_in, int kh, int kw, void *stream);
int az_conv2d_wgrad_bf16(float *grad_w, float *workspace, long long workspace_bytes, const float *grad_out,
                         const float *in, int B, int H, int W, int cm, int cn, int cm_real, int cn_real,
                         int go_cstride, int in_cstride, void *stream);
int az_conv2d_wgrad_f16(float *grad_w, float *workspace, long long workspace_bytes, const float *grad_out,
                        const float *in, const float *go_amax, const float *in_amax, int B, int H, int W,
                        int cm, int cn, int cm_real, int cn_real, int go_cstride, int in_cstride, int kh,
                        int kw, int dilation, void *stream);
int az_conv2d_roll_pack_f16(float *packed, const float *w, const float *w_amax, int cin, int cout,
                            long long stride_out, long long stride_in, int flip, void *stream);
int az_conv2d_roll_fwd_f16(float *out, const float *in, const float *packed, const float *in_amax,
                           const float *w_amax, const float *scale, const float *shift, const float *residual,
                           int relu, int B, int H, int W, int cin, int cout, void *stream);
int az_conv2d_roll_fwd_stats_f16(float *out, float *partials, float *counts, const float *in, const float *packed,
                                 const float *in_amax, const float *w_amax, int groups, int B, int H, int W,
                                 int cin, int cout, void *stream);

int az_conv3d_c1_fwd(float *logits, const float *in, const float *w, const float *addend,
                     const float *in_scale, const float *in_shift, int B, int D, int H, int W, void *stream);
int az_conv3d_c1_dgrad(float *grad_in, const float *grad_logits, const float *w, int B, int D,
                       int H, int W, void *stream);
int az_conv3d_c1_wgrad(float *grad_w, const float *in, const float *grad_logits, const float *in_scale,
                       const float *in_shift, int B, int D, int H, int W, void *stream);
int az_conv3d_c1_plan(long long *plan , int B, int D, int H, int W);

long long az_bn3d_finalize_scratch(int C);
int az_bn3d_finalize(float *mean, float *invstd, float *scale, float *shift,
                     float *running_mean, float *running_var, const float *partials,
                     const float *counts, const float *gamma, const float *beta,
                     long long ntiles, int C, float eps, float momentum,
                     long long *num_batches_tracked, float *scratch, long long scratch_floats, void *stream);
long long az_bn3d_stats_tiles(long long nvox, int C);
int az_bn3d_stats(float *partials, float *counts, const float *x, long long nvox, int C, void *stream);
long long az_bn2d_workspace(int groups, long long nvox, int C);
int az_bn2d_fwd(float *y, float *mean, float *invstd, float *scale, float *shift, float *running_mean,
                float *running_var, const float *x, const float *residual, const float *gamma,
                const float *beta, float *workspace, long long workspace_bytes, int relu, int groups,
                long long nvox, int C, float eps, float momentum, long long *num_batches_tracked ,
                const float *partials, const float *counts, long long partial_tiles ,
                float *y_amax , void *stream);
int az_bn2d_bwd(float *dx, float *dz_out, float *dgamma, float *dbeta, float *workspace,
                long long workspace_bytes, const float *dy, const float *y, const float *x,
                const float *mean, const float *invstd, const float *gamma, const float *scale,
                const float *shift, int relu, int groups, long long nvox, int C,
                float *dx_amax , void *stream);
int az_bn3d_eval_affine(float *scale, float *shift, const float *gamma, const float *beta,
                        const float *running_mean, const float *running_var, float eps, int C,
                        void *stream);
int az_bn3d_apply(float *y, const float *x, const float *scale, const float *shift,
                  const float *residual, int relu, long long nvox, int C, float *y_amax, void *stream);
long long az_bn3d_bwd_workspace(long long nvox, int C);
int az_bn3d_bwd(float *dx, float *dz_out, float *dgamma, float *dbeta, float *coef,
                float *workspace, long long workspace_bytes, const float *dy, const float *y,
                const float *x, const float *mean, const float *invstd, const float *gamma,
                const float *scale, const float *shift, int relu, long long nvox, int C,
                float *dx_amax, int split_out, void *stream);
int az_spp_upsample_fwd(float *out, const float *in, int B, int hs, int ws, int H, int W, int C, int out_cstride,
                        void *stream);
long long az_spp_upsample_bwd_workspace(int B, int ws, int H, int C);
int az_spp_upsample_bwd(float *grad_in, float *workspace, long long workspace_bytes, const float *grad_out, int B,
                        int hs, int ws, int H, int W, int C, int gout_cstride, void *stream);
int az_add_relu(float *y, const float *a, const float *b, int relu, long long n, float *y_amax, void *stream);
int az_sum4(float *y, const float *a, const float *b, const float *c, const float *d, long long n,
            void *stream);

long long az_conv2d_packed_floats(int cin, int cout, int kh, int kw);
int az_conv2d_pack_weights(float *packed, const float *w, int cin, int cout, int ci_real, int co_real,
                           long long stride_out, long long stride_in, int kh, int kw, int flip,
                           void *stream);
int az_conv2d_fwd(float *out, const float *in, const float *packed_w, const float *scale,
                  const float *shift, const float *residual, int relu, int B, int H, int W, int cin,
                  int cout, int in_cstride, int out_cstride, int res_cstride, int kh, int kw,
                  int dilation, void *stream);
long long az_conv2d_wgrad_workspace(int cm, int cn, int kh, int kw);
int az_conv2d_wgrad(float *grad_w, float *workspace, long long workspace_bytes, const float *grad_out,
                    const float *in, int B, int H, int W, int cm, int cn, int cm_real, int cn_real,
                    int go_cstride, int in_cstride, int kh, int kw, int dilation, void *stream);
#define AZ_C2W_KERNEL_R16_AR0 0
#define AZ_C2W_KERNEL_R16_AR1 1
#define AZ_C2W_KERNEL_W64 2
#define AZ_C2W_KERNEL_GENERIC 3
int az_conv2d_wgrad_plan(long long *plan , int f16, int B, int H, int W, int cm, int cn, int kh, int kw, int dilation);
long long az_conv2d_stats_tiles(int B, int H, int W, int groups);
int az_conv2d_fwd_stats(float *out, float *partials, float *counts, const float *in, const float *packed_w,
                        int groups, int B, int H, int W, int cin, int cout, int in_cstride, int out_cstride,
                        int kh, int kw, int dilation, void *stream);

long long az_conv2d_roll_packed_floats(int cin, int cout);
int az_conv2d_roll_pack(float *packed, const float *w, int cin, int cout, long long stride_out, long long stride_in,
                        int flip, void *stream);
int az_conv2d_roll_fwd(float *out, const float *in, const float *packed, const float *scale, const float *shift,
                       const float *residual, int relu, int B, int H, int W, int cin, int cout, void *stream);
long long az_conv2d_roll_stats_rows(int groups, int B, int H, int W, int cin, int cout);
int az_conv2d_roll_fwd_stats(float *out, float *partials, float *counts, const float *in, const float *packed,
                             int groups, int B, int H, int W, int cin, int cout, void *stream);
int az_conv2d_pack_weights_bf16(float *packed, const float *w, int cin, int cout, long long stride_out,
                                long long stride_in, int kh, int kw, void *stream);
int az_conv2d_bf16_fwd(float *out, const float *in, const float *packed_w, const float *bias,
                       const float *residual, const float *gate_z, const float *gate_h, int act, int B, int H,
                       int W, int cin, int cout, int in_cstride, int out_cstride, int res_cstride,
                       int z_cstride, int h_cstride, void *stream);
int az_conv2d_pack_weights_h1(float *packed, const float *w, const float *w_amax, int cin, int cout, long long stride_out,
                              long long stride_in, int flip, void *stream);
int az_conv2d_h1_fwd(float *out, const float *in, const float *packed_w, const float *in_amax, const float *w_amax,
                     const float *bias, const float *residual, const float *gate_z, const float *gate_h, int act, int B, int H,
                     int W, int cin, int cout, int in_cstride, int out_cstride, int res_cstride, int z_cstride,
                     int h_cstride, void *stream);
int az_conv2d_wgrad_h1(float *grad_w, float *workspace, long long workspace_bytes, const float *grad_out, const float *in,
                       const float *go_amax, const float *in_amax, int B, int H, int W, int cm, int cn, int cm_real,
                       int cn_real, int go_cstride, int in_cstride, void *stream);
int az_rows_concat(float *dst, long long npix, long long hw, int nsrc, const float *const *srcs, const int *channels,
                   const int *kinds, void *stream);
int az_rows_slice_to_image(float *image, const float *rows, long long npix, long long hw, int ctot, int at, int c, void *stream);
int az_gru_rh(float *rhx, const float *zr, const float *hx, long long npix, int hid, int inp, void *stream);
int az_gru_out(float *hn, const float *zr, const float *q, const float *hx, long long npix, int hid, int inp, void *stream);
int az_gru_bwd1(float *dq_pre, float *dzr, float *dh_acc, const float *g, const float *zr, const float *q, const float *hx,
                long long npix, int hid, int inp, float *dq_amax, float *dzr_amax, void *stream);
int az_gru_bwd2(float *dzr, float *dh_acc, const float *d_rhx, const float *zr, const float *hx, long long npix, int hid, int inp,
                float *dzr_amax, void *stream);
int az_gru_bwd3(float *dh, float *dx, const float *dh_acc, const float *d_rhx, const float *d_hx, long long npix, int hid, int inp,
                void *stream);
int az_im2col_s2k3(float *patches, const float *x, int B, int C, int H, int W, int Kp, void *stream);
int az_col2im_s2k3(float *grad_x, const float *grad_patches, int B, int C, int H, int W, int Kp,
                   void *stream);

long long az_ir_pattern_workspace(int B, int H, int W, int ks);
int az_ir_pattern(float *pattern, float *workspace, long long workspace_bytes, const float *img_ir,
                  const float *img, int B, int H, int W, int ks, float threshold, void *stream);
int az_ir_pattern_mode(float *pattern, float *workspace, long long workspace_bytes, const float *img_ir,
                       const float *img, int B, int H, int W, int ks, float threshold, int mode, void *stream);

long long az_temporal_ir_workspace(int B, int T, int H, int W, int ks);
int az_temporal_ir(float *pattern, float *workspace, long long workspace_bytes, const void *stack,
                   int stack_is_u8, int B, int T, int H, int W, int ks, float threshold, void *stream);

int az_gt_from_right(float *disp_l, float *extra_l, float *keep_s, uint8_t *mask, int32_t *stats, const float *disp_r,
                     const float *extra, const float *keep, int N, int Ce, int Ck, int Hin, int Win, int H, int W,
                     float scale_h, float scale_w, float lo, float hi, void *stream);

int az_error_img(float *out, const float *est, const float *gt, const uint8_t *mask, int kind, float abs_thres,
                 float rel_thres, int layout, int B, int H, int W, void *stream);

long long az_augment_workspace(int B, int H, int W, int ks);
int az_augment(float *out, float *workspace, long long workspace_bytes, const void *img, int img_is_u8,
               const float *params, int B, int H, int W, int ks, int flags, void *stream);

int az_corr1d_volume(float *corr, const float *f1, const float *f2, int B, int C, int H, int W1,
                     int W2, void *stream);
int az_corr1d_volume_bwd(float *grad_f1, float *grad_f2, const float *grad_corr, const float *f1,
                         const float *f2, int B, int C, int H, int W1, int W2, void *stream);
int az_corr1d_pool(float *dst, const float *src, long long rows, int Wsrc, void *stream);
int az_corr1d_pool_bwd(float *grad_src, const float *grad_dst, long long rows, int Wsrc,
                       void *stream);
int az_corr1d_lookup_fwd(float *out, const float *pyr_level, const float *coords, int B, int H,
                         int W1, int W_level, int radius, int level, int ch_offset, int ch_total,
                         void *stream);
int az_corr1d_lookup_bwd(float *grad_pyr_level, const float *grad_out, const float *coords, int B,
                         int H, int W1, int W_level, int radius, int level, int ch_offset,
                         int ch_total, void *stream);
int az_corr1d_lookup_bwd_acc(float *grad_pyr_level, const float *grad_out, const float *coords, int B,
                         int H, int W1, int W_level, int radius, int level, int ch_offset,
                         int ch_total, void *stream);

int az_disp_loss_fwd(double *acc4, const float *pred3, const float *pred2, const float *pred1,
                     const float *gt, const unsigned char *mask, float lo, float hi, long long n,
                     void *stream);
int az_disp_loss_bwd(float *g3, float *g2, float *g1, const float *pred3, const float *pred2,
                     const float *pred1, const float *gt, const unsigned char *mask, float lo,
                     float hi, const float *gloss, const double *acc4, float w3, float w2, float w1,
                     long long n, void *stream);
int az_disp_metrics(double *acc8, const float *disp_gt, const float *depth_gt,
                    const float *disp_pred, const float *depth_pred, const float *focal_x_baseline,
                    const unsigned char *mask, int B, long long per_batch, void *stream);

int az_convex_up_fwd(float *up, const float *flow, const void *mask, int mask_f16, int N, int D, int D_out, int h,
                     int w, int factor, int mask_channels, int sign, void *stream);
long long az_convex_up_bwd_workspace(int N, int D_out, int h, int w);
int az_convex_up_bwd(void *g_mask, float *g_flow, void *workspace, long long workspace_bytes, const float *g_up,
                     const float *flow, const void *mask, int mask_f16, int N, int D, int D_out, int h, int w,
                     int factor, int mask_channels, int sign, void *stream);

int az_seq_loss_fwd(double *acc3, const float *pred, const float *gt, const void *valid, int valid_u8,
                    float max_flow, int tsign, long long n, void *stream);
int az_seq_loss_bwd(float *g_pred, const float *pred, const float *gt, const void *valid, int valid_u8,
                    float max_flow, int tsign, const float *gloss, const double *acc3, float weight, long long n,
                    void *stream);

int az_costconv_edge_width(int D, int W);
int az_costconv_num_classes(int D);
int az_costconv_merge_fwd(float *kl, float *kr, const float *weight, const float *ml, const float *mr, int ncls, void *stream);
int az_costconv_merge_bwd(float *grad_weight, const float *gkl, const float *gkr, const float *ml, const float *mr, int ncls,
                          void *stream);
int az_costconv_assemble_fwd(float *out, const float *F_bulk, const float *F_edge, const float *G, int B,
                             int D, int H, int W, void *stream);
int az_costconv_assemble_bwd(float *dF_bulk, float *dF_edge, float *dG, const float *grad_out, int B, int D,
                             int H, int W, void *stream);

#ifdef __cplusplus
}
#endif
#endif
```

Baseline: 47.76 pairs/s.

## Fuse logits-conv dgrad into the preceding BN backward for 32-channel head

When the final 32-channel conv+BN+ReLU feeds the 1-channel logits conv with deferred affine, the logits backward hands its gradient and weight to the BN node instead of materialising the 32-channel input gradient. A new two-kernel path (reduce, then apply) recomputes the c1 dgrad on the fly from a shared-memory ring while computing the BN backward statistics and the pre-split f16 output. This removes writing and re-reading a full-size 32-channel gradient tensor, but the dgrad stencil is now computed twice. The shared BN prologue and tile helpers move into common headers.

```diff
diff --git a/activezero_amd/conv3d.py b/activezero_amd/conv3d.py
--- a/activezero_amd/conv3d.py
+++ b/activezero_amd/conv3d.py
@@ -368,6 +368,39 @@
     return bool(need_gx or need_gw)
 
 
+def _head_workspace(raw, cout, relu):
+    b, d, h, w, _ = raw.shape
+    n = _lib.lib().az_c1_bn_bwd_workspace(b, d, h, w, cout, int(relu), 1)
+    if n == _lib.CONST["AZ_EUNSUPPORTED"]:
+        return None
+    if n < 0:
+        _lib.check(int(n), "az_c1_bn_bwd_workspace")
+    return int(n)
+
+
+def _head_dy(glw, raw):
+    g, w = glw
+    b, d, h, wd, _ = raw.shape
+    gy = torch.empty_like(raw)
+    with profiler.scope("conv3d_c1_dgrad", bytes=4.0 * (raw.numel() + g.numel()), bound="hbm"):
+        _call("az_conv3d_c1_dgrad", _p(gy), _p(g), _p(w), b, d, h, wd, _stream())
+    return gy
+
+
+def _head_backward(glw, raw, mean, invstd, gamma, scale, shift, cout, ws_bytes):
+    g, w = glw
+    b, d, h, wd, _ = raw.shape
+    dx_raw = torch.empty_like(raw)
+    dgamma, dbeta, coef = g.new_empty(cout), g.new_empty(cout), g.new_empty(cout, 3)
+    ws, dx_amax = g.new_empty(ws_bytes // 4), g.new_empty(AMAX_SLOTS)
+    with profiler.scope("c1_bn_bwd_32", bytes=4.0 * raw.numel() * 3, bound="hbm"):
+        _call("az_c1_bn_bwd", _p(dx_raw), None, _p(dgamma), _p(dbeta), _p(coef), _p(ws), ws_bytes, _p(g), _p(w), _p(raw),
+              _p(mean), _p(invstd), _p(gamma.detach()), _p(scale), _p(shift), 1, 1, b, cout, d, h, wd, _p(dx_amax), _stream())
+    _set_amax(dx_raw, dx_amax)
+    dx_raw.az_split = True
+    return dx_raw, dgamma, dbeta
+
+
 class _ConvBN(torch.autograd.Function):
 
     @staticmethod
@@ -408,6 +441,8 @@
             nvox = raw.numel() // cout
             if defer is not None and relu and residual is None:
                 defer.scale, defer.shift = scale, shift
+                defer.fuse = bool(cout == 32 and arith.bwd16 and PRESPLIT)
+                ctx.head = defer
                 y = raw
             else:
                 y = torch.empty_like(raw)
@@ -430,11 +465,24 @@
     def backward(ctx, gy):
         x, weight, gamma, raw, y, mean, invstd, scale, shift = ctx.saved_tensors
         mode, relu, has_res, cin, cout, arith, training = ctx.cfg
-        gy = _chk(gy.contiguous(), "grad_y")
         nvox = raw.numel() // cout
-        with torch.cuda.device(gy.device):
-            gy = slot_leftover(ctx, gy)
-            if not training:
+        head = getattr(ctx, "head", None)
+        glw = head.take_grad() if head is not None else None
+        with torch.cuda.device(raw.device):
+            split = fused_ws = None
+            if glw is not None:
+                split = arith.bwd16 and PRESPLIT and _presplit_ok(x, raw, mode, cin, cout, ctx.needs_input_grad[0],
+                                                                  ctx.needs_input_grad[1])
+                parked = getattr(ctx, "az_out_slot", None)
+                fused_ws = _head_workspace(raw, cout, relu) if (split and not (parked is not None and parked.parts)) else None
+                if fused_ws is None:
+                    gy, glw = _head_dy(glw, raw), None
+            if glw is None:
+                gy = slot_leftover(ctx, _chk(gy.contiguous(), "grad_y"))
+            if glw is not None:
+                dx_raw, dgamma, dbeta = _head_backward(glw, raw, mean, invstd, gamma, scale, shift, cout, fused_ws)
+                g_res = None
+            elif not training:
                 s_, rm = invstd, mean
                 dz = gy * (y > 0).to(gy.dtype) if relu else gy
                 dbeta = dz.sum(dim=(0, 1, 2, 3))
@@ -451,8 +499,9 @@
                 ws_bytes = lib.az_bn3d_bwd_workspace(nvox, cout)
                 ws = gy.new_empty(ws_bytes // 4)
                 dx_amax = gy.new_empty(AMAX_SLOTS) if arith.bwd16 else None
-                split = arith.bwd16 and PRESPLIT and _presplit_ok(x, raw, mode, cin, cout, ctx.needs_input_grad[0],
-                                                                  ctx.needs_input_grad[1])
+                if split is None:
+                    split = arith.bwd16 and PRESPLIT and _presplit_ok(x, raw, mode, cin, cout, ctx.needs_input_grad[0],
+                                                                      ctx.needs_input_grad[1])
                 with profiler.scope(f"bn3d_bwd_{cout}", bytes=4.0 * raw.numel() * (7 if (relu and y is not None) else 5), bound="hbm"):
                     _call("az_bn3d_bwd", _p(dx_raw), _p(dz), _p(dgamma), _p(dbeta), _p(coef), _p(ws), ws_bytes,
                           _p(gy), _p(y), _p(raw), _p(mean), _p(invstd), _p(gamma.detach()), _p(scale), _p(shift),
@@ -479,10 +528,19 @@
 
     def __init__(self):
         self.scale = self.shift = None
+        self.fuse = False
+        self._grad = None
 
     @property
     def pending(self):
         return self.scale is not None
+
+    def leave_grad(self, g, w):
+        self._grad = (g, w)
+
+    def take_grad(self):
+        glw, self._grad = self._grad, None
+        return glw
 
 
 def conv_bn(x, conv, bn, mode, relu=False, residual=None, arith=None, defer=None):
@@ -509,8 +567,9 @@
 class _ConvLogits(torch.autograd.Function):
 
     @staticmethod
-    def forward(ctx, x, weight, addend, sink, scale=None, shift=None):
+    def forward(ctx, x, weight, addend, sink, scale=None, shift=None, head=None):
         ctx.sink = sink if (sink is not None and sink.owns(weight)) else None
+        ctx.head = head
         x = _chk(x, "x")
         w = _chk(weight.detach().contiguous(), "weight")
         b, d, h, wd, c = _dims(x)
@@ -533,21 +592,23 @@
         b, d, h, wd, _ = _dims(x)
         gx = gw = None
         with torch.cuda.device(g.device):
-            if ctx.needs_input_grad[0]:
-                gx = torch.empty_like(x)
-                with profiler.scope("conv3d_c1_dgrad", bytes=4.0 * (x.numel() + g.numel()), bound="hbm"):
-                    _call("az_conv3d_c1_dgrad", _p(gx), _p(g), _p(w), b, d, h, wd, _stream())
+            if ctx.needs_input_grad[0] and ctx.head is not None and ctx.head.fuse:
+                ctx.head.leave_grad(g, w)
+                gx = g.new_empty(()).expand(x.shape)
+            elif ctx.needs_input_grad[0]:
+                gx = _head_dy((g, w), x)
             if ctx.needs_input_grad[1]:
                 gw = torch.empty_like(w)
                 with overlap.scope(ctx.sink, x, g, gw, scale, shift), \
                         profiler.scope("conv3d_c1_wgrad", bytes=4.0 * (x.numel() + g.numel()), bound="hbm"):
                     _call("az_conv3d_c1_wgrad", _p(gw), _p(x), _p(g), _p(scale), _p(shift), b, d, h, wd, _stream())
-        return gx, gw, (g if ctx.has_add else None), None, None, None
+        return gx, gw, (g if ctx.has_add else None), None, None, None, None
 
 
 def conv_logits(x, conv, addend=None, sink=None, affine=None):
     sc, sh = (affine.scale, affine.shift) if (affine is not None and affine.pending) else (None, None)
-    return _ConvLogits.apply(x, sink.weight(conv.weight) if sink is not None else conv.weight, addend, sink, sc, sh)
+    return _ConvLogits.apply(x, sink.weight(conv.weight) if sink is not None else conv.weight, addend, sink, sc, sh,
+                             affine if sc is not None else None)
 
 
 class _AddRelu(torch.autograd.Function):
diff --git a/activezero_amd/csrc/az_bn3d.hip b/activezero_amd/csrc/az_bn3d.hip
--- a/activezero_amd/csrc/az_bn3d.hip
+++ b/activezero_amd/csrc/az_bn3d.hip
@@ -1,6 +1,7 @@
 #include <stdlib.h>
 
 #include "az_roll_common.h"
+#include "az_bn_bwd_common.h"
 
 __device__ __forceinline__ double bn_wave_sum(double v) {
 #pragma unroll
@@ -109,25 +110,6 @@
     shift[c] = beta[c] - rm[c] * sc;
 }
 
-typedef float az_v4f __attribute__((ext_vector_type(4)));
-template <bool NT>
-__device__ __forceinline__ float4 bn_ld4(const float4 *p) {
-    if (NT) {
-        const az_v4f v = __builtin_nontemporal_load(reinterpret_cast<const az_v4f *>(p));
-        return make_float4(v[0], v[1], v[2], v[3]);
-    }
-    return *p;
-}
-template <bool NT>
-__device__ __forceinline__ void bn_st4(float4 *p, const float4 &o) {
-    if (NT) {
-        const az_v4f v = {o.x, o.y, o.z, o.w};
-        __builtin_nontemporal_store(v, reinterpret_cast<az_v4f *>(p));
-    } else {
-        *p = o;
-    }
-}
-#define BN_NT_BYTES (256LL << 20)
 
 template <int C, bool NT>
 __global__ void __launch_bounds__(256)
@@ -277,7 +259,6 @@
     }
 }
 
-#define BN_BWD_PARTIAL_FLOATS 32768
 template <int C, bool NT>
 __global__ void __launch_bounds__(256)
 bn_bwd_apply_kernel(float4 *__restrict__ dx, float4 *__restrict__ dz_out,
@@ -290,7 +271,6 @@
                     unsigned *__restrict__ amax = nullptr, const unsigned *__restrict__ pmax = nullptr) {
     constexpr int C4 = C / 4;
     unsigned am = 0;
-    float split_scale = 1.f;
     __shared__ float smu[C], sis[C], k0[C], k1[C], k2[C], ssc[C], ssh[C];
     const bool remask = relu && scale != nullptr;
     const int grp = blockIdx.y;
@@ -301,84 +281,8 @@
         if (remask) { scale += grp * C; shift += grp * C; }
     }
     if (remask && threadIdx.x < C) { ssc[threadIdx.x] = scale[threadIdx.x]; ssh[threadIdx.x] = shift[threadIdx.x]; }
-    if (threadIdx.x < C) {
-        smu[threadIdx.x] = mean[threadIdx.x];
-        sis[threadIdx.x] = invstd[threadIdx.x];
-    }
-    constexpr int COLS = C / 2, ROWS = 256 / COLS;
-    static_assert(COLS <= 64 && 64 % COLS == 0, "a partial row must tile a wave");
-    __shared__ float wsum[4][2 * C];
-    const int j = threadIdx.x % COLS, r = threadIdx.x / COLS, wave = threadIdx.x >> 6;
-    const bool writer = blockIdx.x == 0;
-    const int g_lo = (writer && grp == 0) ? 0 : grp, g_hi = (writer && grp == 0) ? (int)gridDim.y : grp + 1;
-    double dg_tot = 0.0, db_tot = 0.0;
-    for (int g = g_lo; g < g_hi; ++g) {
-        const float4 *p4 = reinterpret_cast<const float4 *>(partial) + (size_t)g * nblocks * COLS;
-        double a0 = 0.0, a1 = 0.0, a2 = 0.0, a3 = 0.0;
-        for (int blk = r; blk < nblocks; blk += ROWS) {
-            const float4 v = p4[(size_t)blk * COLS + j];
-            a0 += v.x; a1 += v.y; a2 += v.z; a3 += v.w;
-        }
-#pragma unroll
-        for (int off = COLS; off < 64; off <<= 1) {
-            a0 += __shfl_xor(a0, off); a1 += __shfl_xor(a1, off); a2 += __shfl_xor(a2, off); a3 += __shfl_xor(a3, off);
-        }
-        __syncthreads();
-        if ((threadIdx.x & 63) < COLS) {
-            wsum[wave][4 * j + 0] = (float)a0; wsum[wave][4 * j + 1] = (float)a1;
-            wsum[wave][4 * j + 2] = (float)a2; wsum[wave][4 * j + 3] = (float)a3;
-        }
-        __syncthreads();
-        if (threadIdx.x < C) {
-            const int c = threadIdx.x;
-            const double sa = ((double)wsum[0][2 * c] + (double)wsum[1][2 * c]) + ((double)wsum[2][2 * c] + (double)wsum[3][2 * c]);
-            const double sb = ((double)wsum[0][2 * c + 1] + (double)wsum[1][2 * c + 1]) + ((double)wsum[2][2 * c + 1] + (double)wsum[3][2 * c + 1]);
-            db_tot += sa; dg_tot += sb;
-            if (g == grp) {
-                k0[c] = gamma[c] * sis[c];
-                k1[c] = (float)(sa / nvox);
-                k2[c] = (float)(sb / nvox);
-                if (writer) { coef[c * 3 + 0] = k0[c]; coef[c * 3 + 1] = k1[c]; coef[c * 3 + 2] = k2[c]; }
-            }
-        }
-    }
-    if (writer && grp == 0 && threadIdx.x < C) { dbeta[threadIdx.x] = (float)db_tot; dgamma[threadIdx.x] = (float)dg_tot; }
-    if (pmax) {
-        const uint4 *m4 = reinterpret_cast<const uint4 *>(pmax);
-        uint4 m = make_uint4(0, 0, 0, 0);
-        for (int blk = r; blk < nblocks; blk += ROWS) {
-            const uint4 v = m4[(size_t)blk * COLS + j];
-            m.x = max(m.x, v.x); m.y = max(m.y, v.y); m.z = max(m.z, v.z); m.w = max(m.w, v.w);
-        }
-#pragma unroll
-        for (int off = COLS; off < 64; off <<= 1) {
-            m.x = max(m.x, (unsigned)__shfl_xor((int)m.x, off)); m.y = max(m.y, (unsigned)__shfl_xor((int)m.y, off));
-            m.z = max(m.z, (unsigned)__shfl_xor((int)m.z, off)); m.w = max(m.w, (unsigned)__shfl_xor((int)m.w, off));
-        }
-        __syncthreads();
-        if ((threadIdx.x & 63) < COLS) {
-            wsum[wave][4 * j + 0] = __uint_as_float(m.x); wsum[wave][4 * j + 1] = __uint_as_float(m.y);
-            wsum[wave][4 * j + 2] = __uint_as_float(m.z); wsum[wave][4 * j + 3] = __uint_as_float(m.w);
-        }
-        __syncthreads();
-        float bnd = 0.f;
-        if (threadIdx.x < C) {
-            const int c = threadIdx.x;
-            const float gm = fmaxf(fmaxf(wsum[0][2 * c], wsum[1][2 * c]), fmaxf(wsum[2][2 * c], wsum[3][2 * c]));
-            const float xm = fmaxf(fmaxf(wsum[0][2 * c + 1], wsum[1][2 * c + 1]), fmaxf(wsum[2][2 * c + 1], wsum[3][2 * c + 1]));
-            bnd = fabsf(k0[c]) * (gm + fabsf(k1[c]) + xm * fabsf(k2[c])) * 1.000001f;
-            bnd = bnd < __builtin_inff() ? bnd : 0.f;
-        }
-#pragma unroll
-        for (int off = 32; off > 0; off >>= 1) bnd = fmaxf(bnd, __shfl_xor(bnd, off));
-        __shared__ float bwave[4];
-        if ((threadIdx.x & 63) == 0) bwave[wave] = bnd;
-        __syncthreads();
-        bnd = fmaxf(fmaxf(bwave[0], bwave[1]), fmaxf(bwave[2], bwave[3]));
-        split_scale = az_pow2(az_f16_scale_exp(bnd));
-        if (writer && grp == 0 && threadIdx.x == 0 && amax) amax[0] = __float_as_uint(bnd);
-    }
-    __syncthreads();
+    const float split_scale = bn_bwd_prologue<C>(smu, sis, k0, k1, k2, mean, invstd, coef, partial, nblocks, gamma, dgamma,
+                                                 dbeta, nvox, amax, pmax);
     for (long long i = blockIdx.x * 256LL + threadIdx.x; i < total4; i += gridDim.x * 256LL) {
         const int c = (int)(i % C4) * 4;
         float4 g = bn_ld4<NT>(&dy[i]);
diff --git a/activezero_amd/csrc/az_bn_bwd_common.h b/activezero_amd/csrc/az_bn_bwd_common.h
--- /dev/null
+++ b/activezero_amd/csrc/az_bn_bwd_common.h
@@ -0,0 +1,114 @@
+#pragma once
+#include "az_roll_common.h"
+
+typedef float az_v4f __attribute__((ext_vector_type(4)));
+template <bool NT>
+__device__ __forceinline__ float4 bn_ld4(const float4 *p) {
+    if (NT) {
+        const az_v4f v = __builtin_nontemporal_load(reinterpret_cast<const az_v4f *>(p));
+        return make_float4(v[0], v[1], v[2], v[3]);
+    }
+    return *p;
+}
+template <bool NT>
+__device__ __forceinline__ void bn_st4(float4 *p, const float4 &o) {
+    if (NT) {
+        const az_v4f v = {o.x, o.y, o.z, o.w};
+        __builtin_nontemporal_store(v, reinterpret_cast<az_v4f *>(p));
+    } else {
+        *p = o;
+    }
+}
+#define BN_NT_BYTES (256LL << 20)
+
+#define BN_BWD_PARTIAL_FLOATS 32768
+
+template <int C>
+__device__ __forceinline__ float bn_bwd_prologue(float *smu, float *sis, float *k0, float *k1, float *k2,
+                                                 const float *__restrict__ mean, const float *__restrict__ invstd,
+                                                 float *__restrict__ coef, const float *__restrict__ partial, int nblocks,
+                                                 const float *__restrict__ gamma, float *__restrict__ dgamma,
+                                                 float *__restrict__ dbeta, double nvox, unsigned *__restrict__ amax,
+                                                 const unsigned *__restrict__ pmax) {
+    float split_scale = 1.f;
+    const int grp = blockIdx.y;
+    if (threadIdx.x < C) {
+        smu[threadIdx.x] = mean[threadIdx.x];
+        sis[threadIdx.x] = invstd[threadIdx.x];
+    }
+    constexpr int COLS = C / 2, ROWS = 256 / COLS;
+    static_assert(COLS <= 64 && 64 % COLS == 0, "a partial row must tile a wave");
+    __shared__ float wsum[4][2 * C];
+    const int j = threadIdx.x % COLS, r = threadIdx.x / COLS, wave = threadIdx.x >> 6;
+    const bool writer = blockIdx.x == 0;
+    const int g_lo = (writer && grp == 0) ? 0 : grp, g_hi = (writer && grp == 0) ? (int)gridDim.y : grp + 1;
+    double dg_tot = 0.0, db_tot = 0.0;
+    for (int g = g_lo; g < g_hi; ++g) {
+        const float4 *p4 = reinterpret_cast<const float4 *>(partial) + (size_t)g * nblocks * COLS;
+        double a0 = 0.0, a1 = 0.0, a2 = 0.0, a3 = 0.0;
+        for (int blk = r; blk < nblocks; blk += ROWS) {
+            const float4 v = p4[(size_t)blk * COLS + j];
+            a0 += v.x; a1 += v.y; a2 += v.z; a3 += v.w;
+        }
+#pragma unroll
+        for (int off = COLS; off < 64; off <<= 1) {
+            a0 += __shfl_xor(a0, off); a1 += __shfl_xor(a1, off); a2 += __shfl_xor(a2, off); a3 += __shfl_xor(a3, off);
+        }
+        __syncthreads();
+        if ((threadIdx.x & 63) < COLS) {
+            wsum[wave][4 * j + 0] = (float)a0; wsum[wave][4 * j + 1] = (float)a1;
+            wsum[wave][4 * j + 2] = (float)a2; wsum[wave][4 * j + 3] = (float)a3;
+        }
+        __syncthreads();
+        if (threadIdx.x < C) {
+            const int c = threadIdx.x;
+            const double sa = ((double)wsum[0][2 * c] + (double)wsum[1][2 * c]) + ((double)wsum[2][2 * c] + (double)wsum[3][2 * c]);
+            const double sb = ((double)wsum[0][2 * c + 1] + (double)wsum[1][2 * c + 1]) + ((double)wsum[2][2 * c + 1] + (double)wsum[3][2 * c + 1]);
+            db_tot += sa; dg_tot += sb;
+            if (g == grp) {
+                k0[c] = gamma[c] * sis[c];
+                k1[c] = (float)(sa / nvox);
+                k2[c] = (float)(sb / nvox);
+                if (writer) { coef[c * 3 + 0] = k0[c]; coef[c * 3 + 1] = k1[c]; coef[c * 3 + 2] = k2[c]; }
+            }
+        }
+    }
+    if (writer && grp == 0 && threadIdx.x < C) { dbeta[threadIdx.x] = (float)db_tot; dgamma[threadIdx.x] = (float)dg_tot; }
+    if (pmax) {
+        const uint4 *m4 = reinterpret_cast<const uint4 *>(pmax);
+        uint4 m = make_uint4(0, 0, 0, 0);
+        for (int blk = r; blk < nblocks; blk += ROWS) {
+            const uint4 v = m4[(size_t)blk * COLS + j];
+            m.x = max(m.x, v.x); m.y = max(m.y, v.y); m.z = max(m.z, v.z); m.w = max(m.w, v.w);
+        }
+#pragma unroll
+        for (int off = COLS; off < 64; off <<= 1) {
+            m.x = max(m.x, (unsigned)__shfl_xor((int)m.x, off)); m.y = max(m.y, (unsigned)__shfl_xor((int)m.y, off));
+            m.z = max(m.z, (unsigned)__shfl_xor((int)m.z, off)); m.w = max(m.w, (unsigned)__shfl_xor((int)m.w, off));
+        }
+        __syncthreads();
+        if ((threadIdx.x & 63) < COLS) {
+            wsum[wave][4 * j + 0] = __uint_as_float(m.x); wsum[wave][4 * j + 1] = __uint_as_float(m.y);
+            wsum[wave][4 * j + 2] = __uint_as_float(m.z); wsum[wave][4 * j + 3] = __uint_as_float(m.w);
+        }
+        __syncthreads();
+        float bnd = 0.f;
+        if (threadIdx.x < C) {
+            const int c = threadIdx.x;
+            const float gm = fmaxf(fmaxf(wsum[0][2 * c], wsum[1][2 * c]), fmaxf(wsum[2][2 * c], wsum[3][2 * c]));
+            const float xm = fmaxf(fmaxf(wsum[0][2 * c + 1], wsum[1][2 * c + 1]), fmaxf(wsum[2][2 * c + 1], wsum[3][2 * c + 1]));
+            bnd = fabsf(k0[c]) * (gm + fabsf(k1[c]) + xm * fabsf(k2[c])) * 1.000001f;
+            bnd = bnd < __builtin_inff() ? bnd : 0.f;
+        }
+#pragma unroll
+        for (int off = 32; off > 0; off >>= 1) bnd = fmaxf(bnd, __shfl_xor(bnd, off));
+        __shared__ float bwave[4];
+        if ((threadIdx.x & 63) == 0) bwave[wave] = bnd;
+        __syncthreads();
+        bnd = fmaxf(fmaxf(bwave[0], bwave[1]), fmaxf(bwave[2], bwave[3]));
+        split_scale = az_pow2(az_f16_scale_exp(bnd));
+        if (writer && grp == 0 && threadIdx.x == 0 && amax) amax[0] = __float_as_uint(bnd);
+    }
+    __syncthreads();
+    return split_scale;
+}
diff --git a/activezero_amd/csrc/az_c1_bn_bwd.hip b/activezero_amd/csrc/az_c1_bn_bwd.hip
--- /dev/null
+++ b/activezero_amd/csrc/az_c1_bn_bwd.hip
@@ -0,0 +1,274 @@
+#include "az_bn_bwd_common.h"
+#include "az_c1_tile.h"
+
+#define C1BN_TH 8
+#define C1BN_TW 16
+#define C1BN_SY (C1BN_TH + 2)
+#define C1BN_SX (C1BN_TW + 2)
+#define C1BN_GP 20
+#define C1BN_RING 4
+#define C1BN_PLANE (C1BN_SY * C1BN_GP)
+static_assert(C1BN_SY * C1BN_SX <= 256, "one halo value per thread");
+
+struct c1bn_patch { int b, ty0, tx0; };
+__device__ __forceinline__ float c1bn_fetch(const float *__restrict__ gout, const c1bn_patch &pt, int gd, int D, int H, int W) {
+    const int sy = threadIdx.x / C1BN_SX, sx = threadIdx.x - sy * C1BN_SX;
+    const int gh = pt.ty0 - 1 + sy, gw = pt.tx0 - 1 + sx;
+    return (sy < C1BN_SY && gd >= 0 && gd < D && gh >= 0 && gh < H && gw >= 0 && gw < W)
+               ? gout[(((size_t)pt.b * D + gd) * H + gh) * W + gw] : 0.f;
+}
+__device__ __forceinline__ void c1bn_commit(float *ring, int gd, float v) {
+    const int sy = threadIdx.x / C1BN_SX, sx = threadIdx.x - sy * C1BN_SX;
+    if (sy < C1BN_SY) ring[(gd & (C1BN_RING - 1)) * C1BN_PLANE + sy * C1BN_GP + sx] = v;
+}
+template <bool NT>
+__device__ __forceinline__ unsigned c1bn_load_x4(float4 (&x)[4], const float *__restrict__ in, const c1bn_patch &pt, int od,
+                                                 int ih, int iw0, int D, int H, int W, int quad) {
+    unsigned ok = 0;
+    const float *src = in + ((((size_t)pt.b * D + od) * H + ih) * W + iw0) * 32 + quad * 4;
+#pragma unroll
+    for (int j = 0; j < 4; ++j) {
+        x[j] = make_float4(0.f, 0.f, 0.f, 0.f);
+        if (ih < H && iw0 + j < W) {
+            x[j] = bn_ld4<NT>(reinterpret_cast<const float4 *>(src + j * 32));
+            ok |= 1u << j;
+        }
+    }
+    return ok;
+}
+__device__ __forceinline__ void c1bn_dz4(float4 (&dz)[4], const float4 (&x)[4], unsigned ok4, const float *ring, int od,
+                                         int ly, int lx0, const c1_f2 (&w01)[27], const c1_f2 (&w23)[27],
+                                         const float4 &sc, const float4 &sh) {
+    c1_f2 a01[4], a23[4];
+#pragma unroll
+    for (int j = 0; j < 4; ++j) { a01[j] = c1_f2{0.f, 0.f}; a23[j] = c1_f2{0.f, 0.f}; }
+#pragma unroll
+    for (int kd = 0; kd < 3; ++kd)
+#pragma unroll
+        for (int kh = 0; kh < 3; ++kh) {
+            const float *row = static_cast<const float *>(__builtin_assume_aligned(
+                ring + ((od + 1 - kd) & (C1BN_RING - 1)) * C1BN_PLANE + (ly + 2 - kh) * C1BN_GP + lx0, 16));
+            const float4 ra = *reinterpret_cast<const float4 *>(row);
+            const float2 rb = *reinterpret_cast<const float2 *>(row + 4);
+            const float r[6] = {ra.x, ra.y, ra.z, ra.w, rb.x, rb.y};
+#pragma unroll
+            for (int kw = 0; kw < 3; ++kw) {
+                const int t = (kd * 3 + kh) * 3 + kw;
+#pragma unroll
+                for (int j = 0; j < 4; ++j) {
+                    const c1_f2 g2 = {r[j + 2 - kw], r[j + 2 - kw]};
+                    a01[j] = C1_FMA2(g2, w01[t], a01[j]);
+                    a23[j] = C1_FMA2(g2, w23[t], a23[j]);
+                }
+            }
+        }
+#pragma unroll
+    for (int j = 0; j < 4; ++j) asm volatile("" : "+v"(a01[j]), "+v"(a23[j]));
+#pragma unroll
+    for (int j = 0; j < 4; ++j) {
+        const bool in = (ok4 >> j) & 1u;
+        dz[j].x = (in && fmaf(x[j].x, sc.x, sh.x) > 0.f) ? a01[j][0] : 0.f;
+        dz[j].y = (in && fmaf(x[j].y, sc.y, sh.y) > 0.f) ? a01[j][1] : 0.f;
+        dz[j].z = (in && fmaf(x[j].z, sc.z, sh.z) > 0.f) ? a23[j][0] : 0.f;
+        dz[j].w = (in && fmaf(x[j].w, sc.w, sh.w) > 0.f) ? a23[j][1] : 0.f;
+    }
+}
+template <bool NT, class F>
+__device__ __forceinline__ void c1bn_walk(float *ring, const float *__restrict__ in, const float *__restrict__ gout,
+                                          const float *__restrict__ w, const float *__restrict__ scale,
+                                          const float *__restrict__ shift, int D, int H, int W, int tiles_x, int tiles_y,
+                                          long long nplanes, long long chunk, F &&consume) {
+    const int quad = threadIdx.x & 7, grp = threadIdx.x >> 3, ly = grp >> 2, lx0 = (grp & 3) * 4;
+    const float4 sc = reinterpret_cast<const float4 *>(scale)[quad], sh = reinterpret_cast<const float4 *>(shift)[quad];
+    c1_f2 w01[27], w23[27];
+#pragma unroll
+    for (int t = 0; t < 27; ++t) {
+        w01[t] = c1_f2{w[(quad * 4 + 0) * 27 + t], w[(quad * 4 + 1) * 27 + t]};
+        w23[t] = c1_f2{w[(quad * 4 + 2) * 27 + t], w[(quad * 4 + 3) * 27 + t]};
+    }
+    long long at = blockIdx.x * chunk;
+    const long long end = min(at + chunk, nplanes);
+    while (at < end) {
+        long long r = at / D;
+        const int d0 = (int)(at - r * D), d1 = (int)min((long long)D, d0 + (end - at));
+        c1bn_patch pt;
+        pt.tx0 = (int)(r % tiles_x) * C1BN_TW; r /= tiles_x;
+        pt.ty0 = (int)(r % tiles_y) * C1BN_TH;
+        pt.b = (int)(r / tiles_y);
+        at += d1 - d0;
+        const int ih = pt.ty0 + ly, iw0 = pt.tx0 + lx0;
+        const float g0 = c1bn_fetch(gout, pt, d0 - 1, D, H, W), g1 = c1bn_fetch(gout, pt, d0, D, H, W);
+        float gn = c1bn_fetch(gout, pt, d0 + 1, D, H, W);
+        float4 xn[4];
+        unsigned okn = c1bn_load_x4<NT>(xn, in, pt, d0, ih, iw0, D, H, W, quad);
+        __syncthreads();
+        c1bn_commit(ring, d0 - 1, g0);
+        c1bn_commit(ring, d0, g1);
+#pragma unroll 1
+        for (int od = d0; od < d1; ++od) {
+            c1bn_commit(ring, od + 1, gn);
+            __syncthreads();
+            float4 x[4];
+#pragma unroll
+            for (int j = 0; j < 4; ++j) x[j] = xn[j];
+            const unsigned ok = okn;
+            if (od + 1 < d1) {
+                gn = c1bn_fetch(gout, pt, od + 2, D, H, W);
+                okn = c1bn_load_x4<NT>(xn, in, pt, od + 1, ih, iw0, D, H, W, quad);
+            }
+            float4 dz[4];
+            c1bn_dz4(dz, x, ok, ring, od, ly, lx0, w01, w23, sc, sh);
+            consume(x, dz, ok, ((((size_t)pt.b * D + od) * H + ih) * W + iw0) * 32 + quad * 4);
+        }
+    }
+}
+
+template <bool NT>
+__global__ void __launch_bounds__(256, 2)
+c1bn_reduce_kernel(float *__restrict__ partial, unsigned *__restrict__ pmax, unsigned *__restrict__ amax_zero,
+                   const float *__restrict__ in, const float *__restrict__ gout, const float *__restrict__ w,
+                   const float *__restrict__ mean, const float *__restrict__ invstd, const float *__restrict__ scale,
+                   const float *__restrict__ shift, int D, int H, int W, int tiles_x, int tiles_y,
+                   long long nplanes, long long chunk) {
+    __shared__ __attribute__((aligned(16))) float ring[C1BN_RING * C1BN_PLANE];
+    if (blockIdx.x == 0 && threadIdx.x < AZ_AMAX_SLOTS) amax_zero[threadIdx.x * AZ_AMAX_STRIDE] = 0u;
+    const int quad = threadIdx.x & 7;
+    const float4 mu = reinterpret_cast<const float4 *>(mean)[quad], is = reinterpret_cast<const float4 *>(invstd)[quad];
+    float4 s1 = make_float4(0, 0, 0, 0), s2 = make_float4(0, 0, 0, 0);
+    uint4 mg = make_uint4(0, 0, 0, 0), mx = make_uint4(0, 0, 0, 0);
+    c1bn_walk<NT>(ring, in, gout, w, scale, shift, D, H, W, tiles_x, tiles_y, nplanes, chunk,
+                  [&](const float4 (&x)[4], const float4 (&dz)[4], unsigned ok, size_t) {
+#pragma unroll
+        for (int j = 0; j < 4; ++j) {
+            if (!((ok >> j) & 1u)) continue;
+            const float4 xx = x[j], g = dz[j];
+            const float4 xh = make_float4((xx.x - mu.x) * is.x, (xx.y - mu.y) * is.y, (xx.z - mu.z) * is.z, (xx.w - mu.w) * is.w);
+            s1.x += g.x; s1.y += g.y; s1.z += g.z; s1.w += g.w;
+            s2.x += g.x * xh.x; s2.y += g.y * xh.y; s2.z += g.z * xh.z; s2.w += g.w * xh.w;
+            mg.x = max(mg.x, az_finite_abs_bits(g.x)); mg.y = max(mg.y, az_finite_abs_bits(g.y));
+            mg.z = max(mg.z, az_finite_abs_bits(g.z)); mg.w = max(mg.w, az_finite_abs_bits(g.w));
+            mx.x = max(mx.x, az_finite_abs_bits(xh.x)); mx.y = max(mx.y, az_finite_abs_bits(xh.y));
+            mx.z = max(mx.z, az_finite_abs_bits(xh.z)); mx.w = max(mx.w, az_finite_abs_bits(xh.w));
+        }
+    });
+#pragma unroll
+    for (int off = 8; off < 64; off <<= 1) {
+        s1.x += __shfl_xor(s1.x, off); s1.y += __shfl_xor(s1.y, off); s1.z += __shfl_xor(s1.z, off); s1.w += __shfl_xor(s1.w, off);
+        s2.x += __shfl_xor(s2.x, off); s2.y += __shfl_xor(s2.y, off); s2.z += __shfl_xor(s2.z, off); s2.w += __shfl_xor(s2.w, off);
+        mg.x = max(mg.x, (unsigned)__shfl_xor((int)mg.x, off)); mg.y = max(mg.y, (unsigned)__shfl_xor((int)mg.y, off));
+        mg.z = max(mg.z, (unsigned)__shfl_xor((int)mg.z, off)); mg.w = max(mg.w, (unsigned)__shfl_xor((int)mg.w, off));
+        mx.x = max(mx.x, (unsigned)__shfl_xor((int)mx.x, off)); mx.y = max(mx.y, (unsigned)__shfl_xor((int)mx.y, off));
+        mx.z = max(mx.z, (unsigned)__shfl_xor((int)mx.z, off)); mx.w = max(mx.w, (unsigned)__shfl_xor((int)mx.w, off));
+    }
+    __shared__ float4 r1[4][8], r2[4][8];
+    __shared__ uint4 q1[4][8], q2[4][8];
+    const int wave = threadIdx.x >> 6, lane = threadIdx.x & 63;
+    if (lane < 8) { r1[wave][lane] = s1; r2[wave][lane] = s2; q1[wave][lane] = mg; q2[wave][lane] = mx; }
+    __syncthreads();
+    if (threadIdx.x < 8) {
+#pragma unroll
+        for (int k = 1; k < 4; ++k) {
+            const float4 a = r1[k][quad], b = r2[k][quad];
+            const uint4 c = q1[k][quad], d = q2[k][quad];
+            s1.x += a.x; s1.y += a.y; s1.z += a.z; s1.w += a.w;
+            s2.x += b.x; s2.y += b.y; s2.z += b.z; s2.w += b.w;
+            mg.x = max(mg.x, c.x); mg.y = max(mg.y, c.y); mg.z = max(mg.z, c.z); mg.w = max(mg.w, c.w);
+            mx.x = max(mx.x, d.x); mx.y = max(mx.y, d.y); mx.z = max(mx.z, d.z); mx.w = max(mx.w, d.w);
+        }
+        float *p = partial + ((size_t)blockIdx.x * 32 + quad * 4) * 2;
+        p[0] = s1.x; p[1] = s2.x; p[2] = s1.y; p[3] = s2.y;
+        p[4] = s1.z; p[5] = s2.z; p[6] = s1.w; p[7] = s2.w;
+        unsigned *m = pmax + ((size_t)blockIdx.x * 32 + quad * 4) * 2;
+        m[0] = mg.x; m[1] = mx.x; m[2] = mg.y; m[3] = mx.y;
+        m[4] = mg.z; m[5] = mx.z; m[6] = mg.w; m[7] = mx.w;
+    }
+}
+
+template <bool NT>
+__global__ void __launch_bounds__(256, 2)
+c1bn_apply_kernel(float *__restrict__ dx, float *__restrict__ dz_out, const float *__restrict__ in,
+                  const float *__restrict__ gout, const float *__restrict__ w, const float *__restrict__ mean,
+                  const float *__restrict__ invstd, float *__restrict__ coef, const float *__restrict__ scale,
+                  const float *__restrict__ shift, const float *__restrict__ partial, int nblocks,
+                  const float *__restrict__ gamma, float *__restrict__ dgamma, float *__restrict__ dbeta, double nvox,
+                  unsigned *__restrict__ amax, const unsigned *__restrict__ pmax, int D, int H, int W, int tiles_x,
+                  int tiles_y, long long nplanes, long long chunk) {
+    __shared__ __attribute__((aligned(16))) float ring[C1BN_RING * C1BN_PLANE];
+    __shared__ __attribute__((aligned(16))) float smu[32], sis[32], k0[32], k1[32], k2[32];
+    const float split_scale = bn_bwd_prologue<32>(smu, sis, k0, k1, k2, mean, invstd, coef, partial, nblocks, gamma, dgamma,
+                                                  dbeta, nvox, amax, pmax);
+    const int quad = threadIdx.x & 7;
+    const float4 mu = reinterpret_cast<const float4 *>(smu)[quad], is = reinterpret_cast<const float4 *>(sis)[quad];
+    const float4 c0 = reinterpret_cast<const float4 *>(k0)[quad], c1 = reinterpret_cast<const float4 *>(k1)[quad];
+    const float4 c2 = reinterpret_cast<const float4 *>(k2)[quad];
+    c1bn_walk<NT>(ring, in, gout, w, scale, shift, D, H, W, tiles_x, tiles_y, nplanes, chunk,
+                  [&](const float4 (&x)[4], const float4 (&dz)[4], unsigned ok, size_t o) {
+#pragma unroll
+        for (int j = 0; j < 4; ++j) {
+            if (!((ok >> j) & 1u)) continue;
+            const float4 xx = x[j], g = dz[j];
+            if (dz_out) bn_st4<NT>(reinterpret_cast<float4 *>(dz_out + o + j * 32), g);
+            float4 r;
+            r.x = c0.x * (g.x - c1.x - (xx.x - mu.x) * is.x * c2.x);
+            r.y = c0.y * (g.y - c1.y - (xx.y - mu.y) * is.y * c2.y);
+            r.z = c0.z * (g.z - c1.z - (xx.z - mu.z) * is.z * c2.z);
+            r.w = c0.w * (g.w - c1.w - (xx.w - mu.w) * is.w * c2.w);
+            bn_st4<NT>(reinterpret_cast<float4 *>(dx + o + j * 32),
+                       az_presplit_f16x4(make_float4(r.x * split_scale, r.y * split_scale, r.z * split_scale, r.w * split_scale)));
+        }
+    });
+}
+
+static long long c1bn_planes(int B, int D, int H, int W) {
+    return (long long)B * D * ((H + C1BN_TH - 1) / C1BN_TH) * ((W + C1BN_TW - 1) / C1BN_TW);
+}
+static int c1bn_blocks(long long nplanes, int cap) {
+    const long long chunk = (nplanes + cap - 1) / cap;
+    return (int)((nplanes + chunk - 1) / chunk);
+}
+#define C1BN_REDUCE_CAP (BN_BWD_PARTIAL_FLOATS / (2 * 32))
+#define C1BN_APPLY_CAP 1024
+static int c1bn_check(int B, int D, int H, int W, int C, int relu, int groups) {
+    if (!(B > 0 && D > 0 && H > 0 && W > 0 && C > 0 && groups > 0)) return AZ_EINVAL;
+    if (C != 32 || !relu || groups != 1) return AZ_EUNSUPPORTED;
+    if ((long long)B * D * H * W * 32 > 0x7fffffffLL) return AZ_EUNSUPPORTED;
+    return AZ_OK;
+}
+
+extern "C" long long az_c1_bn_bwd_workspace(int B, int D, int H, int W, int C, int relu, int groups) {
+    if (int e = c1bn_check(B, D, H, W, C, relu, groups)) return e;
+    return 2LL * c1bn_blocks(c1bn_planes(B, D, H, W), C1BN_REDUCE_CAP) * 32 * 2 * (long long)sizeof(float);
+}
+
+extern "C" int az_c1_bn_bwd(float *dx, float *dz_out, float *dgamma, float *dbeta, float *coef, float *workspace,
+                            long long workspace_bytes, const float *grad_logits, const float *w, const float *x,
+                            const float *mean, const float *invstd, const float *gamma, const float *scale,
+                            const float *shift, int relu, int groups, int B, int C, int D, int H, int W, float *dx_amax,
+                            void *stream) {
+    if (int e = c1bn_check(B, D, H, W, C, relu, groups)) return e;
+    AZ_REQUIRE_PTR(dx); AZ_REQUIRE_PTR(dgamma); AZ_REQUIRE_PTR(dbeta); AZ_REQUIRE_PTR(coef); AZ_REQUIRE_PTR(workspace);
+    AZ_REQUIRE_PTR(grad_logits); AZ_REQUIRE_PTR(w); AZ_REQUIRE_PTR(x); AZ_REQUIRE_PTR(mean); AZ_REQUIRE_PTR(invstd);
+    AZ_REQUIRE_PTR(gamma); AZ_REQUIRE_PTR(scale); AZ_REQUIRE_PTR(shift); AZ_REQUIRE_PTR(dx_amax);
+    if (workspace_bytes < az_c1_bn_bwd_workspace(B, D, H, W, C, relu, groups)) return AZ_EWORKSPACE;
+    const int tiles_x = (W + C1BN_TW - 1) / C1BN_TW, tiles_y = (H + C1BN_TH - 1) / C1BN_TH;
+    const long long nplanes = c1bn_planes(B, D, H, W), nvox = (long long)B * D * H * W;
+    const int blocks = c1bn_blocks(nplanes, C1BN_REDUCE_CAP), agrid = c1bn_blocks(nplanes, C1BN_APPLY_CAP);
+    const long long rchunk = (nplanes + blocks - 1) / blocks, achunk = (nplanes + agrid - 1) / agrid;
+    unsigned *const am = reinterpret_cast<unsigned *>(dx_amax);
+    unsigned *const pmax = reinterpret_cast<unsigned *>(workspace) + (size_t)blocks * 32 * 2;
+    hipStream_t s = az_stream(stream);
+    if (nvox * 32 * 4 >= BN_NT_BYTES) {
+        hipLaunchKernelGGL(c1bn_reduce_kernel<true>, dim3(blocks), dim3(256), 0, s, workspace, pmax, am, x, grad_logits, w, mean,
+                           invstd, scale, shift, D, H, W, tiles_x, tiles_y, nplanes, rchunk);
+        hipLaunchKernelGGL(c1bn_apply_kernel<true>, dim3(agrid), dim3(256), 0, s, dx, dz_out, x, grad_logits, w, mean, invstd, coef,
+                           scale, shift, (const float *)workspace, blocks, gamma, dgamma, dbeta, (double)nvox, am,
+                           (const unsigned *)pmax, D, H, W, tiles_x, tiles_y, nplanes, achunk);
+    } else {
+        hipLaunchKernelGGL(c1bn_reduce_kernel<false>, dim3(blocks), dim3(256), 0, s, workspace, pmax, am, x, grad_logits, w, mean,
+                           invstd, scale, shift, D, H, W, tiles_x, tiles_y, nplanes, rchunk);
+        hipLaunchKernelGGL(c1bn_apply_kernel<false>, dim3(agrid), dim3(256), 0, s, dx, dz_out, x, grad_logits, w, mean, invstd, coef,
+                           scale, shift, (const float *)workspace, blocks, gamma, dgamma, dbeta, (double)nvox, am,
+                           (const unsigned *)pmax, D, H, W, tiles_x, tiles_y, nplanes, achunk);
+    }
+    return az_launch_status();
+}
diff --git a/activezero_amd/csrc/az_c1_tile.h b/activezero_amd/csrc/az_c1_tile.h
--- /dev/null
+++ b/activezero_amd/csrc/az_c1_tile.h
@@ -0,0 +1,16 @@
+#pragma once
+#include "az_common.h"
+
+#define C1_TH 8
+#define C1_TW 32
+#define C1_VS 36
+#define C1_GP 36
+typedef float c1_f2 __attribute__((ext_vector_type(2)));
+#define C1_FMA2(a, b, c) __builtin_elementwise_fma(a, b, c)
+
+__device__ __forceinline__ void c1_row6(float (&r)[6], const float *gt, int pd, int sy, int lx0) {
+    const float *row = static_cast<const float *>(__builtin_assume_aligned(gt + (pd * (C1_TH + 2) + sy) * C1_GP + lx0, 16));
+    const float4 a = *reinterpret_cast<const float4 *>(row);
+    const float2 c = *reinterpret_cast<const float2 *>(row + 4);
+    r[0] = a.x; r[1] = a.y; r[2] = a.z; r[3] = a.w; r[4] = c.x; r[5] = c.y;
+}
diff --git a/activezero_amd/csrc/az_conv3d_c1.hip b/activezero_amd/csrc/az_conv3d_c1.hip
--- a/activezero_amd/csrc/az_conv3d_c1.hip
+++ b/activezero_amd/csrc/az_conv3d_c1.hip
@@ -1,12 +1,6 @@
 #include "az_common.h"
 #include "az_launch_math.h"
-
-#define C1_TH 8
-#define C1_TW 32
-#define C1_VS 36
-#define C1_GP 36
-typedef float c1_f2 __attribute__((ext_vector_type(2)));
-#define C1_FMA2(a, b, c) __builtin_elementwise_fma(a, b, c)
+#include "az_c1_tile.h"
 
 
 #define C1F_TH 8
@@ -127,12 +121,6 @@
         gt[r * C1_GP + sx] = (gd >= 0 && gd < D && gh >= 0 && gh < H && gw >= 0 && gw < W)
                                  ? gout[(((size_t)b * D + gd) * H + gh) * W + gw] : 0.f;
     }
-}
-__device__ __forceinline__ void c1_row6(float (&r)[6], const float *gt, int pd, int sy, int lx0) {
-    const float *row = static_cast<const float *>(__builtin_assume_aligned(gt + (pd * (C1_TH + 2) + sy) * C1_GP + lx0, 16));
-    const float4 a = *reinterpret_cast<const float4 *>(row);
-    const float2 c = *reinterpret_cast<const float2 *>(row + 4);
-    r[0] = a.x; r[1] = a.y; r[2] = a.z; r[3] = a.w; r[4] = c.x; r[5] = c.y;
 }
 
 __global__ void __launch_bounds__(256)
diff --git a/include/azhip.h b/include/azhip.h
--- a/include/azhip.h
+++ b/include/azhip.h
@@ -187,6 +187,12 @@
                 const float *x, const float *mean, const float *invstd, const float *gamma,
                 const float *scale, const float *shift, int relu, long long nvox, int C,
                 float *dx_amax, int split_out, void *stream);
+long long az_c1_bn_bwd_workspace(int B, int D, int H, int W, int C, int relu, int groups);
+int az_c1_bn_bwd(float *dx, float *dz_out, float *dgamma, float *dbeta, float *coef, float *workspace,
+                 long long workspace_bytes, const float *grad_logits, const float *w, const float *x,
+                 const float *mean, const float *invstd, const float *gamma, const float *scale,
+                 const float *shift, int relu, int groups, int B, int C, int D, int H, int W, float *dx_amax,
+                 void *stream);
 int az_spp_upsample_fwd(float *out, const float *in, int B, int hs, int ws, int H, int W, int C, int out_cstride,
                         void *stream);
 long long az_spp_upsample_bwd_workspace(int B, int ws, int H, int C);
```

Result: no change. 48.08 pairs/s, median of 6 (+0.7%).
